# jalberse/RayTracingInOneWeekendInRust

Measured on AMD Instinct MI355X. Metric: Msamples/s (rays traced/s) + HBM GB/s vs roofline, showcase@1200x800x500spp, higher is better.
Workload: dtype f32; 1 GPU; C3 showcase 1200x800 500spp depth 50; scene=showcase, width=1200, height=800, spp=500, max_depth=50, parallelism=one GPU: the whole frame, exact_bvh=False

## Files before the change

### raytracinginoneweekendinrust_amd/__init__.py

```python
from __future__ import annotations

import ctypes as C
from dataclasses import dataclass, field
from typing import List, Optional, Sequence, Tuple

import numpy as np

from . import _capi
from ._capi import ASSET_DIR, RTError, check, lib
from .configs import CONFIGS, RenderConfig

__all__ = ["Camera", "CameraBasis", "BvhNode", "Renderer", "Scene", "SceneBuilder", "HittableList", "DeviceScene", "RenderConfig", "CONFIGS",
           "RTError", "tile", "device_count", "numeric_eval", "scene_background", "render_params", "ASSET_DIR",
           "set_option", "get_option", "options"]

Vec3 = Tuple[float, float, float]


class Scene:

    def __init__(self, desc_ptr, owner=None, name: str = ""):
        self._ptr = desc_ptr
        self._owner = owner
        self._lib_owned = owner is None
# ... 336 lines not shown
        yield done, (acc.copy() if last else acc / np.float32(done))


def render_multi(scenes: List[DeviceScene], camera: Camera, params,
                 out: Optional[np.ndarray] = None) -> Tuple[np.ndarray, dict]:
    if out is None:
        out = np.zeros((params.height, params.width, 3), dtype=np.float32)
    assert out.dtype == np.float32 and out.flags.c_contiguous and out.size == params.width * params.height * 3
    handles = (C.c_void_p * len(scenes))(*[s.handle for s in scenes])
    st = _capi.rt_stats()
    cam = camera.desc()
    check(lib.rt_render_multi(handles, len(scenes), C.byref(cam), C.byref(params),
                              out.ctypes.data_as(C.POINTER(C.c_float)), C.byref(st)), "rt_render_multi")
    return out, {"segments": st.segments, "samples": st.samples, "kernel_ms": st.kernel_ms}


def shard_floats(width: int, height: int, rank: int, n: int) -> int:
    return int(lib.rt_shard_floats(width, height, rank, n))


def shard_offset(width: int, height: int, rank: int, n: int) -> int:
    return int(lib.rt_shard_offset(width, height, rank, n))


def shard_mask(width: int, height: int, rank: int, n: int, device=None):
    import torch
    y = torch.arange(height, device=device).view(-1, 1) // 8
    x = torch.arange(width, device=device).view(1, -1) // 8
    return ((y * ((width + 7) // 8) + x) % n == rank).reshape(-1)


def shard_pack(d_image, width: int, height: int, rank: int, n: int, d_packed, stream: int = 0) -> None:
    check(lib.rt_shard_pack(C.c_void_p(d_image.data_ptr()), width, height, rank, n, C.c_void_p(d_packed.data_ptr()),
                            C.c_void_p(stream or None)), "rt_shard_pack")


IPC_HANDLE_BYTES = 72


def ipc_export(d_ptr: int, device: int) -> bytes:
    h = C.create_string_buffer(IPC_HANDLE_BYTES)
    check(lib.rt_ipc_export(C.c_void_p(d_ptr), device, h), "rt_ipc_export")
    return h.raw


def ipc_open(handle: bytes, device: int) -> int:
    p = C.c_void_p()
    check(lib.rt_ipc_open(C.create_string_buffer(handle, IPC_HANDLE_BYTES), device, C.byref(p)), "rt_ipc_open")
    return int(p.value)


def ipc_close(d_ptr: int, device: int) -> None:
    check(lib.rt_ipc_close(C.c_void_p(d_ptr), device), "rt_ipc_close")


def copy_async(d_dst: int, d_src: int, nbytes: int, stream: int = 0) -> None:
    check(lib.rt_copy_async(C.c_void_p(d_dst), C.c_void_p(d_src), nbytes, C.c_void_p(stream or None)),
          "rt_copy_async")


def shard_pull_unpack(peer_ptrs, width: int, height: int, d_image, stream: int = 0) -> None:
    n = len(peer_ptrs)
    arr = (C.c_void_p * n)(*[p or None for p in peer_ptrs])
    check(lib.rt_shard_pull_unpack(arr, width, height, n, C.c_void_p(d_image.data_ptr()), C.c_void_p(stream or None)),
          "rt_shard_pull_unpack")


def shard_unpack(d_packed_all, width: int, height: int, n: int, d_image, stream: int = 0) -> None:
    check(lib.rt_shard_unpack(C.c_void_p(d_packed_all.data_ptr()), width, height, n, C.c_void_p(d_image.data_ptr()),
                              C.c_void_p(stream or None)), "rt_shard_unpack")


def format_ppm(img: np.ndarray, device: int = 0) -> bytes:
    import torch
    h, w, _ = img.shape
    d_img = torch.from_numpy(np.ascontiguousarray(img, dtype=np.float32)).to(f"cuda:{device}")
    d_txt = torch.empty(12 * w * h, dtype=torch.uint8, device=f"cuda:{device}")
    n = C.c_uint64()
    stream = torch.cuda.current_stream(device).cuda_stream
    check(lib.rt_format_ppm(C.c_void_p(d_img.data_ptr()), w, h, C.c_void_p(d_txt.data_ptr()), d_txt.numel(),
                            C.byref(n), C.c_void_p(stream or None)), "rt_format_ppm")
    return f"P3\n{w} {h}\n255\n".encode() + bytes(d_txt[: n.value].cpu().numpy())


def quantize_srgb8(img: np.ndarray, device: int = 0) -> np.ndarray:
    import torch
    h, w, _ = img.shape
    d_img = torch.from_numpy(np.ascontiguousarray(img, dtype=np.float32)).to(f"cuda:{device}")
    d_u8 = torch.empty(3 * w * h, dtype=torch.uint8, device=f"cuda:{device}")
    stream = torch.cuda.current_stream(device).cuda_stream
    check(lib.rt_quantize_srgb8(C.c_void_p(d_img.data_ptr()), C.c_void_p(d_u8.data_ptr()), w, h,
                                C.c_void_p(stream or None)), "rt_quantize_srgb8")
    return d_u8.cpu().numpy().reshape(h, w, 3)


def tile(image_width: int, image_height: int, tile_width: int, tile_height: int) -> List[Tuple[int, int, int, int]]:
    n = C.c_uint32()
    check(lib.rt_tile_image(image_width, image_height, tile_width, tile_height, None, 0, C.byref(n)), "rt_tile_image")
    arr = (_capi.rt_tile * max(n.value, 1))()
    check(lib.rt_tile_image(image_width, image_height, tile_width, tile_height, arr, n.value, C.byref(n)),
          "rt_tile_image")
    return [(t.width, t.height, t.x_start, t.y_start) for t in arr[: n.value]]


def set_option(name: str, value: int) -> None:
    check(lib.rt_set_option(_capi.OPTIONS[name], int(value)), f"rt_set_option({name})")


def get_option(name: str) -> int:
    v = C.c_int64()
    check(lib.rt_get_option(_capi.OPTIONS[name], C.byref(v)), f"rt_get_option({name})")
    return v.value


class options:

    def __init__(self, **kw):
        self.kw = kw
        self.saved = {}

    def __enter__(self):
        for k, v in self.kw.items():
            self.saved[k] = get_option(k)
            set_option(k, v)
        return self

    def __exit__(self, *exc):
        for k, v in self.saved.items():
            set_option(k, v)
        return False


def device_count() -> int:
    n = C.c_int()
    check(lib.rt_device_count(C.byref(n)), "rt_device_count")
    return n.value


def scene_background(name: str) -> Vec3:
    rgb = (C.c_float * 3)()
    check(lib.rt_scene_background(name.encode(), rgb), "rt_scene_background")
    return (rgb[0], rgb[1], rgb[2])


def device_kat(op: int, cases) -> np.ndarray:
    a = np.ascontiguousarray(cases, dtype=np.float32)
    n = a.shape[0]
    out = np.zeros((n, 2), dtype=np.float32)
    check(lib.rt_device_kat(op, a.ctypes.data_as(C.POINTER(C.c_float)), out.ctypes.data_as(C.POINTER(C.c_float)), n),
          "rt_device_kat")
    return out


def numeric_eval(op: int, a: np.ndarray, b: Optional[np.ndarray] = None) -> np.ndarray:
    a = np.ascontiguousarray(a, dtype=np.float64)
    out = np.empty_like(a)
    bp = None
    if b is not None:
        b = np.ascontiguousarray(b, dtype=np.float64)
        bp = b.ctypes.data_as(C.POINTER(C.c_double))
    check(lib.rt_device_numeric_eval(op, a.ctypes.data_as(C.POINTER(C.c_double)), bp,
                                      out.ctypes.data_as(C.POINTER(C.c_double)), a.size), "rt_device_numeric_eval")
    return out
```

### raytracinginoneweekendinrust_amd/csrc/kernel.hip

```cpp
#include <hip/hip_runtime.h>
#include <stdint.h>
#include <stdio.h>
#include <math.h>
#include <stdlib.h>
#include <string.h>

#include <algorithm>
#include <atomic>
#include <mutex>
#include <string>
#include <vector>

#include "../../include/rt.h"
#include "../../include/rt_numeric_spec.h"
#include "common.hpp"
#include "device_scene.hpp"
#include "lower.hpp"

using rtdev::DevCamera;
using rtdev::DevEntry;
using rtdev::DevMaterial;
using rtdev::DevParams;
using rtdev::DevScene;
using rtdev::DevTexture;
using rtdev::f4;

#define RT_DEV __device__ __forceinline__

namespace {

constexpr float kInf = __builtin_inff();

enum ProfRegion : uint32_t {
    kPrRefill = 0, kPrSegment, kPrWorld, kPrRecord, kPrEmit, kPrScatter, kPrMarble, kPrStore,
    kPrChecker, kPrImage, kPrUnitSphere, kPrDielectric, kPrLambert, kPrMetal, kPrIso, kPrLog,
    kPrEntry0 = 16, kPrEntryLast = 43, kPrBvhTrip = 44, kPrLeafTest = 45, kPrBvhSetup = 46, kPrBvhPush = 47,
    kPrBvhPop = 48, kPrBvhCall = 49, kPrCount = 52
};
constexpr uint32_t kModeExact = 1u, kModeNoLeafBoxes = 2u, kModeNoPermLds = 32u, kModeW3 = 64u,
                   kModeNoPretest = 128u, kModeReplayRef = 1u << 16;
constexpr uint32_t kModeNoStream = 1u << 17;
constexpr uint32_t kModePruneAllExp = 1u << 20;
#if defined(RT_LEAF_AUDIT) || defined(RT_ABLATE)
constexpr bool kPruneAllExpBuild = true;
#else
constexpr bool kPruneAllExpBuild = false;
#endif
constexpr uint32_t kModeBlocksForward = 1u << 21;
constexpr uint32_t kModeW4 = 1u << 22;
[[maybe_unused]] constexpr uint32_t kModeMbShrink = 1u << 29;
constexpr uint32_t kTuneExact = kModeNoLeafBoxes | kModeNoPermLds | kModeW3 | kModeNoPretest | kModeReplayRef |
                                kModeNoStream | kModeBlocksForward | kModeW4 | (15u << 24);
constexpr uint32_t kTuneAccepted = kTuneExact
#if defined(RT_LEAF_AUDIT) || defined(RT_ABLATE)
                                   | kModePruneAllExp
#endif
#ifdef RT_LEAF_AUDIT
                                   | kModeMbShrink
#endif
#ifdef RT_ABLATE
                                   | (31u << 8)
#endif
#ifdef RT_EXP_STRIDE
                                   | (1u << 23)
#endif
    ;
#ifdef RT_ABLATE
constexpr uint32_t kAbLeaf2 = 1u << 8, kAbKeys2 = 1u << 9, kAbBvh2 = 1u << 10, kAbMedium2 = 1u << 11,
                   kAbGeom2 = 1u << 12;
#define ABLATE(bit, ...) do { if (mode & (bit)) { __VA_ARGS__ } } while (0)
#else
#define ABLATE(bit, ...) do { } while (0)
#endif
#ifdef RT_PROFILE_REGIONS
constexpr uint32_t kProfCopies = 64;
constexpr uint32_t kProfWords = 3 * kPrCount + 16;
__device__ unsigned long long g_prof[kProfCopies * kProfWords];
constexpr uint32_t kProfWaves = 8192;
__device__ unsigned long long g_wave_t[2 * kProfWaves];
constexpr uint32_t kTpBuckets = 4096, kTpTicks = 20000u;
__device__ unsigned long long g_tp_hist[kTpBuckets];
constexpr uint32_t kRoleEvents = 4096;
__device__ unsigned long long g_role_ev[2 * kRoleEvents];
__device__ unsigned g_role_n;
uint32_t g_prof_rows[2] = {0u, 0xffffffffu};
__device__ __forceinline__ void role_event(uint32_t what) {
    const unsigned i = atomicAdd(&g_role_n, 1u);
    if (i < kRoleEvents) {
        g_role_ev[2u * i] = __builtin_amdgcn_s_memrealtime();
        g_role_ev[2u * i + 1u] = what;
    }
}
__shared__ unsigned long long prof_lds[kProfWords];
__device__ __forceinline__ uint32_t trips_bin(uint32_t n) {
    return n == 0u ? 0u : n == 1u ? 1u : n == 2u ? 2u : n <= 4u ? 3u : n <= 8u ? 4u : n <= 16u ? 5u : n <= 32u ? 6u : 7u;
}
__device__ __forceinline__ void prof_init() {
    for (uint32_t i = threadIdx.x; i < kProfWords; i += blockDim.x) prof_lds[i] = 0u;
}
__device__ __forceinline__ void prof_flush() {
    unsigned long long* dst = g_prof + (blockIdx.x % kProfCopies) * kProfWords;
    for (uint32_t i = threadIdx.x; i < kProfWords; i += blockDim.x)
        if (prof_lds[i]) atomicAdd(&dst[i], prof_lds[i]);
}
#define PROF_T0(name) const uint64_t name = __builtin_amdgcn_s_memtime()
#define PROF_ADD(region, t0) prof_add((region), (t0))
__device__ __forceinline__ void prof_add(uint32_t region, uint64_t t0) {
    uint64_t dt = __builtin_amdgcn_s_memtime() - t0;
    uint64_t m = __ballot(1);
    if (__lane_id() == (uint32_t)__builtin_ctzll(m)) {
        prof_lds[region] += dt;
        prof_lds[kPrCount + region] += 1u;
        prof_lds[2 * kPrCount + region] += (uint64_t)__popcll(m);
    }
}
#define PROF_INIT() prof_init()
#define PROF_FLUSH() prof_flush()
#else
#define PROF_T0(name) do { } while (0)
#define PROF_ADD(region, t0) do { } while (0)
#define PROF_INIT() do { } while (0)
#define PROF_FLUSH() do { } while (0)
#endif
#ifdef RT_LEAF_AUDIT
struct LeafAudit {
    float o[3], d[3], tmin, closest, t, box[6], delta;
    uint32_t code, rank, best_rank;
};
constexpr uint32_t kAuditMax = 64;
__device__ unsigned g_audit_count;
__device__ LeafAudit g_audit[kAuditMax];
struct TravAudit {
    float o[3], d[3], tmin, tmax, fast_t, ref_t;
    uint32_t fast_code, ref_code, root;
};
__device__ unsigned g_trav_audit_count;
__device__ unsigned g_bounds_audit_count;
__device__ TravAudit g_trav_audit[kAuditMax];
#endif

struct V {
    float x, y, z;
};
#ifdef RT_DEBUG_PIXEL
constexpr uint32_t kDbgMax = 256;
__device__ uint32_t g_dbg[8 * kDbgMax];
__device__ unsigned g_dbg_n;
#ifndef RT_DEBUG_TRACE
#define RT_DEBUG_TRACE 1
#endif
#ifdef RT_DEBUG_INLINE
__device__ __forceinline__
#else
__device__ __noinline__
#endif
void dbg_put(uint32_t tag, uint32_t a, uint32_t b, uint32_t c, uint32_t d, uint32_t e,
                                     uint32_t f, uint32_t h) {
    const unsigned i = atomicAdd(&g_dbg_n, 1u);
    if (i < kDbgMax) {
        uint32_t* o = g_dbg + 8u * i;
        o[0] = tag; o[1] = a; o[2] = b; o[3] = c; o[4] = d; o[5] = e; o[6] = f; o[7] = h;
    }
}
#endif
RT_DEV V mk(float x, float y, float z) { return V{x, y, z}; }
RT_DEV V operator+(V a, V b) { return V{a.x + b.x, a.y + b.y, a.z + b.z}; }
RT_DEV V operator-(V a, V b) { return V{a.x - b.x, a.y - b.y, a.z - b.z}; }
RT_DEV V operator*(V a, V b) { return V{a.x * b.x, a.y * b.y, a.z * b.z}; }
RT_DEV V operator*(float s, V a) { return V{s * a.x, s * a.y, s * a.z}; }
RT_DEV V operator-(V a) { return V{-a.x, -a.y, -a.z}; }
RT_DEV V divs(V a, float s) { return V{a.x / s, a.y / s, a.z / s}; }
RT_DEV float dot(V a, V b) { return (a.x * b.x + a.y * b.y) + a.z * b.z; }
RT_DEV V cross(V a, V b) { return V{a.y * b.z - b.y * a.z, a.z * b.x - b.z * a.x, a.x * b.y - b.x * a.y}; }
RT_DEV float length(V a) { return __builtin_sqrtf(dot(a, a)); }
RT_DEV V normalize(V a) {
    float r = 1.0f / length(a);
    return V{a.x * r, a.y * r, a.z * r};
}
RT_DEV float rs_min(float a, float b) {
    if (a != a) return b;
    if (b != b) return a;
    return a < b ? a : b;
}
RT_DEV float rs_clamp(float x, float lo, float hi) {
    if (x < lo) x = lo;
    if (x > hi) x = hi;
    return x;
}
RT_DEV bool sign_negative(float x) { return (__float_as_uint(x) >> 31) != 0u; }
RT_DEV bool sign_negative_d(double x) { return (__double_as_longlong(x) >> 63) != 0; }
RT_DEV V xyz(f4 a) { return V{a.x, a.y, a.z}; }
[[maybe_unused]] RT_DEV float2 ld2(const f4* p, uint32_t row) {
    float2 v;
    __builtin_memcpy(&v, __builtin_assume_aligned(p + row, 16), sizeof(v));
    return v;
}
RT_DEV f4 ld4(const f4* p) {
    f4 v;
    __builtin_memcpy(&v, __builtin_assume_aligned(p, 16), sizeof(v));
    return v;
}
RT_DEV f4 ld4_at(const f4* base, uint32_t byte_off) {
    f4 v;
    __builtin_memcpy(&v, __builtin_assume_aligned(reinterpret_cast<const char*>(base) + byte_off, 16), sizeof(v));
    return v;
}
RT_DEV float ld1_at(const f4* base, uint32_t byte_off) {
    float v;
    __builtin_memcpy(&v, __builtin_assume_aligned(reinterpret_cast<const char*>(base) + byte_off, 4), sizeof(v));
    return v;
}
RT_DEV float2 ld2_at(const f4* base, uint32_t byte_off) {
    float2 v;
    __builtin_memcpy(&v, __builtin_assume_aligned(reinterpret_cast<const char*>(base) + byte_off, 8), sizeof(v));
    return v;
}
#ifndef RT_SCALAR_ENTRIES
#define RT_SCALAR_ENTRIES 1
#endif
#if RT_SCALAR_ENTRIES
#define RT_AS4 __attribute__((address_space(4)))
#else
#define RT_AS4
#endif
template <class T>
RT_DEV const RT_AS4 T* cst(const T* p) {
    return (const RT_AS4 T*)p;
}
RT_DEV f4 ld4c(const f4* p) {
    const RT_AS4 f4* q = cst(p);
    return f4{q->x, q->y, q->z, q->w};
}

struct Ray {
    V o, d;
    float time;
};
RT_DEV V at(const Ray& r, float t) { return r.o + t * r.d; }

struct Rng {
    uint32_t sample, pixel, d;
    uint32_t r0, r1, r2;
};
RT_DEV void philox(uint32_t& c0, uint32_t& c1, uint32_t& c2, uint32_t& c3, uint32_t k0, uint32_t k1) {
#pragma unroll
    for (int r = 0; r < 10; ++r) {
        const uint64_t p0 = (uint64_t)0xD2511F53u * c0, p1 = (uint64_t)0xCD9E8D57u * c2;
        const uint32_t lo0 = (uint32_t)p0, hi0 = (uint32_t)(p0 >> 32), lo1 = (uint32_t)p1, hi1 = (uint32_t)(p1 >> 32);
        uint32_t n0 = hi1 ^ c1 ^ k0, n2 = hi0 ^ c3 ^ k1;
        c0 = n0; c1 = lo1; c2 = n2; c3 = lo0;
        k0 += 0x9E3779B9u;
        k1 += 0xBB67AE85u;
    }
}
struct Key {
    uint32_t k0, k1;
};

#ifdef RT_PHILOX_CALL
__device__ __noinline__
#else
__device__ __forceinline__
#endif
uint4 philox_block(uint32_t c0, uint32_t c1, uint32_t c2, uint32_t k0, uint32_t k1) {
    uint32_t c3 = 0u;
    philox(c0, c1, c2, c3, k0, k1);
    return make_uint4(c0, c1, c2, c3);
}
#ifndef RT_RNG_UNIFORM
#ifdef RT_PHILOX_CALL
#define RT_RNG_UNIFORM 1
#else
#define RT_RNG_UNIFORM 0
#endif
#endif
// ... 546 lines not shown
            k = atomicCAS(&sl->key, ~0ull, key);
            if (k == ~0ull || k == key) return sl;
        }
    }
    return nullptr;
}
RT_DEV uint32_t hrpp_leaf_node(const DevScene& S, unsigned long long k) {
    uint32_t lo = 0, hi = S.hrpp_nkeys;
    while (lo < hi) {
        const uint32_t m = (lo + hi) >> 1;
        if (S.hrpp_keys[m] < k) lo = m + 1;
        else hi = m;
    }
    return lo < S.hrpp_nkeys && S.hrpp_keys[lo] == k ? S.hrpp_vals[lo] : 0xffffffffu;
}
RT_DEV bool bvh_hit_hrpp(const DevScene& S, uint32_t wrapper2, uint32_t pid, const Ray& r,
                                          const RayD& q, V inv, float tmin, float& closest, uint32_t& hit_code,
                                          uint32_t* stk) {
    rtdev::HrppSlot* tab = S.hrpp_tab + ((size_t)(pid - 1u) << S.hrpp_bits);
    uint32_t* cnt = S.hrpp_cnt + 4u * (pid - 1u);
    const unsigned long long key = hrpp_hash(r);
    const rtdev::HrppSlot* sl = S.hrpp_bits ? hrpp_find(tab, S.hrpp_bits, key, false) : nullptr;
    bool predicted = false;
    if (sl) {
        float c = closest;
        uint32_t code = 0u;
        bool any = false;
        for (uint32_t j = 0; j < rtdev::kHrppIds; ++j) {
            const uint32_t w = __hip_atomic_load(&sl->ids[j], __ATOMIC_RELAXED, __HIP_MEMORY_SCOPE_AGENT);
            if (w == 0xffffffffu) break;
            predicted = true;
            if (bvh_hit_reference(S, w, r, q, inv, tmin, c, code, stk)) any = true;
        }
        if (any) {
            atomicAdd(&cnt[0], 1u);
            closest = c;
            hit_code = code;
            return true;
        }
    }
    atomicAdd(&cnt[predicted ? 1u : 2u], 1u);
    const bool h = bvh_hit_reference(S, wrapper2, r, q, inv, tmin, closest, hit_code, stk);
    if (h && S.hrpp_bits) {
        const uint32_t leaf = hrpp_leaf_node(S, (unsigned long long)wrapper2 << 32 | hit_code);
        rtdev::HrppSlot* ins = leaf != 0xffffffffu ? hrpp_find(tab, S.hrpp_bits, key, true) : nullptr;
        bool ok = false;
        if (ins)
            for (uint32_t j = 0; j < rtdev::kHrppIds && !ok; ++j) {
                const uint32_t old = atomicCAS(&ins->ids[j], 0xffffffffu, leaf);
                ok = old == 0xffffffffu || old == leaf;
            }
        if (!ok) atomicAdd(&cnt[3], 1u);
    }
    return h;
}

[[maybe_unused]] RT_DEV float child_key(float x0, float y0, float z0, float x1, float y1, float z1, const Ray& r, V inv, float tmin,
                       float tmax_entry, float closest, bool prune, float dmi) {
    float te;
    bool go = slab(x0, y0, z0, x1, y1, z1, r, inv, tmin, tmax_entry, te);
    if (prune) te = te - dmi;
    if (go && prune) go = !(te > prune_bound(closest));
    return go ? (te < 3.4028235e38f ? te : 3.4028235e38f) : kInf;
}
typedef float pk2 __attribute__((ext_vector_type(2)));
RT_DEV pk2 pk(float a, float b) { return pk2{a, b}; }
RT_DEV void child_keys4_nf(f4 nx, f4 ny, f4 nz, f4 fx, f4 fy, f4 fz, const Ray& r, V inv, float tmin,
                           float tmax_entry, float pb, float dmi, float key[4]) {
    const pk2 ox = pk(r.o.x, r.o.x), oy = pk(r.o.y, r.o.y), oz = pk(r.o.z, r.o.z);
    const pk2 ix = pk(inv.x, inv.x), iy = pk(inv.y, inv.y), iz = pk(inv.z, inv.z);
#pragma unroll
    for (int h = 0; h < 2; ++h) {
        const pk2 tnx = ((h ? pk(nx.z, nx.w) : pk(nx.x, nx.y)) - ox) * ix, tfx = ((h ? pk(fx.z, fx.w) : pk(fx.x, fx.y)) - ox) * ix;
        const pk2 tny = ((h ? pk(ny.z, ny.w) : pk(ny.x, ny.y)) - oy) * iy, tfy = ((h ? pk(fy.z, fy.w) : pk(fy.x, fy.y)) - oy) * iy;
        const pk2 tnz = ((h ? pk(nz.z, nz.w) : pk(nz.x, nz.y)) - oz) * iz, tfz = ((h ? pk(fz.z, fz.w) : pk(fz.x, fz.y)) - oz) * iz;
#pragma unroll
        for (int e = 0; e < 2; ++e) {
            const float lo = __builtin_fmaxf(__builtin_fmaxf(tnx[e], tny[e]), __builtin_fmaxf(tnz[e], tmin));
            const float hi = __builtin_fminf(__builtin_fminf(tfx[e], tfy[e]), __builtin_fminf(tfz[e], tmax_entry));
            const float te = lo - dmi;
            const bool go = lo <= hi && te <= pb;
            key[2 * h + e] = go ? __builtin_fminf(te, 3.4028235e38f) : kInf;
        }
    }
}
RT_DEV void leaf_intervals2_nf(float2 nx, float2 ny, float2 nz, float2 fx, float2 fy, float2 fz, const Ray& r,
                               V inv, float delta, float lo[2], float hi[2]) {
    const bool sx = inv.x < 0.0f, sy = inv.y < 0.0f, sz = inv.z < 0.0f;
    const float pxs = r.o.x + delta, pys = r.o.y + delta, pzs = r.o.z + delta;
    const float mxs = r.o.x - delta, mys = r.o.y - delta, mzs = r.o.z - delta;
    const float anx = sx ? mxs : pxs, afx = sx ? pxs : mxs, sny = sy ? mys : pys, afy = sy ? pys : mys;
    const float anz = sz ? mzs : pzs, afz = sz ? pzs : mzs;
    const pk2 ix = pk(inv.x, inv.x), iy = pk(inv.y, inv.y), iz = pk(inv.z, inv.z);
    const pk2 tnx = (pk(nx.x, nx.y) - pk(anx, anx)) * ix, tfx = (pk(fx.x, fx.y) - pk(afx, afx)) * ix;
    const pk2 tny = (pk(ny.x, ny.y) - pk(sny, sny)) * iy, tfy = (pk(fy.x, fy.y) - pk(afy, afy)) * iy;
    const pk2 tnz = (pk(nz.x, nz.y) - pk(anz, anz)) * iz, tfz = (pk(fz.x, fz.y) - pk(afz, afz)) * iz;
#pragma unroll
    for (int e = 0; e < 2; ++e) {
        lo[e] = __builtin_fmaxf(__builtin_fmaxf(tnx[e], tny[e]), tnz[e]);
        hi[e] = __builtin_fminf(__builtin_fminf(tfx[e], tfy[e]), tfz[e]);
    }
}
RT_DEV bool leaf_interval_may_hit(float lo, float hi, float tmin, float closest) {
    if (lo > prune_bound(closest)) return false;
    if (tmin > 0.0f && hi < tmin * (1.0f - 0x1p-19f)) return false;
    return !(lo - hi > (__builtin_fabsf(lo) + __builtin_fabsf(hi)) * 0x1p-19f);
}
RT_DEV void sort2(float& ta, uint32_t& ca, float& tb, uint32_t& cb) {
    const bool sw = tb < ta;
    const float a = ta, b = tb;
    const uint32_t x = ca, y = cb;
    ta = sw ? b : a;
    tb = sw ? a : b;
    ca = sw ? y : x;
    cb = sw ? x : y;
}
struct Trav {
    uint32_t cur, sp, best_rank;
    float tmax_entry;
    bool any;
    uint32_t pend;
};
constexpr uint32_t kNoNode = 0xffffffffu;
RT_DEV void trav_audit(const DevScene& S, const f4* wrapper, uint32_t root, const Ray& r, V inv, float tmin,
                       const Trav& tv, float closest, uint32_t hit_code, uint32_t* stk) {
#ifdef RT_LEAF_AUDIT
    const bool any = tv.any;
    float c2 = tv.tmax_entry;
    uint32_t h2 = 0u;
    bool a2 = bvh_hit_reference(S, __float_as_uint(ld4c(wrapper + 7).z), r, to_d(r), inv, tmin, c2, h2, stk);
    bool same = a2 == any && (!any || (__float_as_uint(c2) == __float_as_uint(closest) && h2 == hit_code));
    if (!same) {
        unsigned i_ = atomicAdd(&g_trav_audit_count, 1u);
        if (i_ < kAuditMax) {
            TravAudit& A = g_trav_audit[i_];
            A.o[0] = r.o.x; A.o[1] = r.o.y; A.o[2] = r.o.z;
            A.d[0] = r.d.x; A.d[1] = r.d.y; A.d[2] = r.d.z;
            A.tmin = tmin; A.tmax = tv.tmax_entry;
            A.fast_t = any ? closest : kInf; A.ref_t = a2 ? c2 : kInf;
            A.fast_code = any ? hit_code : 0xffffffffu; A.ref_code = a2 ? h2 : 0xffffffffu;
            A.root = root;
        }
    }
#endif
}
#ifndef RT_SUSP_MIN_TRIPS
#define RT_SUSP_MIN_TRIPS 2
#endif
constexpr uint32_t kSuspMinTrips = RT_SUSP_MIN_TRIPS;
#ifndef RT_LEAF_Q
#define RT_LEAF_Q 8
#endif

template <int kKind, uint32_t kF, bool kSusp>
RT_DEV bool bvh_run(const DevScene& S, float delta, const f4* wrapper, const Ray& r, V inv, float tmin, float& closest,
                    uint32_t& hit_code, uint32_t* stk, uint32_t mode, Trav& tv, uint32_t susp);
constexpr uint32_t kRayFast = 0u, kRayHandOver = 1u, kRayNoHit = 2u;
#ifndef RT_TRI_ZERO_DIR_FAST
#define RT_TRI_ZERO_DIR_FAST 1
#endif
template <int kKind, uint32_t kF>
RT_DEV uint32_t ray_route(const Ray& r, V inv, float tmax_entry, const f4* wrapper, uint32_t mode) {
    const float ax = __builtin_fabsf(inv.x), ay = __builtin_fabsf(inv.y), az = __builtin_fabsf(inv.z);
    const bool ofin = __builtin_fabsf(r.o.x) < kInf && __builtin_fabsf(r.o.y) < kInf && __builtin_fabsf(r.o.z) < kInf;
    const bool tnum = tmax_entry == tmax_entry;
    if (ax > 0.0f && ax < kInf && ay > 0.0f && ay < kInf && az > 0.0f && az < kInf && ofin && tnum) return kRayFast;
    if constexpr ((kF & kFTri) != 0u && (kKind == 3 || (kKind == 0 && RT_TRI_ZERO_DIR_FAST))) {
        if ((__float_as_uint(ld4c(wrapper + 7).w) & rtdev::kBvhTriOnly) != 0u &&
            !(kPruneAllExpBuild && (mode & kModePruneAllExp))) {
            if (r.o.x != r.o.x || r.o.y != r.o.y || r.o.z != r.o.z || r.d.x != r.d.x || r.d.y != r.d.y ||
                r.d.z != r.d.z)
                return kRayNoHit;
            const bool dfin =
                __builtin_fabsf(r.d.x) < kInf && __builtin_fabsf(r.d.y) < kInf && __builtin_fabsf(r.d.z) < kInf;
            if (dfin && ofin && tnum) return kRayFast;
        }
    }
    return kRayHandOver;
}

template <uint32_t kF>
RT_DEV bool bvh_hit_nan_tmax(const DevScene& S, const f4* wrapper, const Ray& r, float tmin, float& closest,
                             uint32_t& hit_code) {
    const f4* T = S.nodes + (size_t)__float_as_uint(ld4c(wrapper + 7).y) * rtdev::kBvhNodeF4;
    const uint32_t n = __float_as_uint(ld1_at(T, 0u));
    const float nan = __uint_as_float(0x7fc00000u);
    bool any = false;
    float best = 0.0f;
    uint32_t best_code = 0u;
    auto test = [&](uint32_t i, float tmax, float& t) {
        const uint32_t idx = rtdev::leaf_index(__float_as_uint(ld1_at(T, 16u + 4u * i)));
        return tri_t(ld4(S.tri + 3 * (size_t)idx), ld4(S.tri + 3 * (size_t)idx + 1), ld4(S.tri + 3 * (size_t)idx + 2), r,
                     tmin, tmax, t);
    };
    for (uint32_t i = 0; i < n;) {
        const uint32_t e = __float_as_uint(ld1_at(T, 16u + 4u * i));
        const bool pair = (e & rtdev::kDfsPairLeft) != 0u && i + 1u < n;
        float tl = 0.0f, tr = 0.0f;
        const bool hl = test(i, nan, tl);
        const bool hr = pair && test(i + 1u, hl ? tl : nan, tr);
        if (hl || hr) {
            const float t = hr ? tr : tl;
            if (!any || !(best < t)) {
                any = true;
                best = t;
                best_code = __float_as_uint(ld1_at(T, 16u + 4u * (hr ? i + 1u : i))) & ~rtdev::kDfsPairLeft;
            }
        }
        i += pair ? 2u : 1u;
    }
    if (!any) return false;
    closest = best;
    hit_code = best_code;
    return true;
}

#ifndef RT_PEEL_WRAPPER
#define RT_PEEL_WRAPPER 1
#endif
constexpr bool kPeelWrapper = RT_PEEL_WRAPPER;
template <int kKind, uint32_t kF = kFAll>
RT_DEV bool bvh_hit(const DevScene& S, float delta, uint32_t root, const Ray& r, float tmin, float& closest,
                    uint32_t& hit_code, uint32_t* stk, uint32_t mode, bool& replay) {
    PROF_T0(pcall);
    PROF_T0(psetup);
    const f4* wrapper = S.nodes + (size_t)root * rtdev::kBvhNodeF4;
    const V inv = mk(1.0f / r.d.x, 1.0f / r.d.y, 1.0f / r.d.z);
    if constexpr (kKind == 1 || kKind == 2) {
        const RayD q = to_d(r);
        const uint32_t w2 = __float_as_uint(ld4c(wrapper + 7).z);
        if constexpr (kKind == 2) {
            const uint32_t pid = __float_as_uint(S.nodes2[4 * (size_t)w2 + 3].z);
            if (pid) return bvh_hit_hrpp(S, w2, pid, r, q, inv, tmin, closest, hit_code, stk);
        }
        return bvh_hit_reference(S, w2, r, q, inv, tmin, closest, hit_code, stk);
    }
    {
        const uint32_t route = ray_route<kKind, kF>(r, inv, closest, wrapper, mode);
        if (route == kRayNoHit) return false;
        if constexpr (kKind == 3) {
            if (route == kRayHandOver) {
                if constexpr ((kF & kFTri) != 0u) {
                    const bool fin = __builtin_fabsf(r.o.x) < kInf && __builtin_fabsf(r.o.y) < kInf &&
                                     __builtin_fabsf(r.o.z) < kInf && __builtin_fabsf(r.d.x) < kInf &&
                                     __builtin_fabsf(r.d.y) < kInf && __builtin_fabsf(r.d.z) < kInf;
                    if (closest != closest && fin &&
                        (__float_as_uint(ld4c(wrapper + 7).w) & rtdev::kBvhTriOnly) != 0u &&
                        !(kPruneAllExpBuild && (mode & kModePruneAllExp)))
                        return bvh_hit_nan_tmax<kF>(S, wrapper, r, tmin, closest, hit_code);
                }
                return bvh_hit_reference(S, __float_as_uint(ld4c(wrapper + 7).z), r, to_d(r), inv, tmin, closest, hit_code,
                                         stk);
            }
        }
        if (route == kRayHandOver) {
            replay = true;
            return false;
        }
    }
    PROF_ADD(kPrBvhSetup, psetup);
    Trav tv{root, 0u, 0u, closest, false, kNoNode};
    if constexpr (kPeelWrapper) {
        const f4 w0 = ld4c(wrapper), w1 = ld4c(wrapper + 1), w2 = ld4c(wrapper + 2), w3 = ld4c(wrapper + 3),
                 w4 = ld4c(wrapper + 4), w5 = ld4c(wrapper + 5), w6 = ld4c(wrapper + 6), w7 = ld4c(wrapper + 7);
        const bool prune = (__float_as_uint(w7.w) & rtdev::kBvhPrunable) != 0u ||
                           (kPruneAllExpBuild && (mode & kModePruneAllExp));
        const float dmi = delta * fmaxf(fmaxf(__builtin_fabsf(inv.x), __builtin_fabsf(inv.y)), __builtin_fabsf(inv.z));
        const bool sx = inv.x < 0.0f, sy = inv.y < 0.0f, sz = inv.z < 0.0f;
        const float tnx = ((sx ? w3.x : w0.x) - r.o.x) * inv.x, tfx = ((sx ? w0.x : w3.x) - r.o.x) * inv.x;
        const float tny = ((sy ? w4.x : w1.x) - r.o.y) * inv.y, tfy = ((sy ? w1.x : w4.x) - r.o.y) * inv.y;
        const float tnz = ((sz ? w5.x : w2.x) - r.o.z) * inv.z, tfz = ((sz ? w2.x : w5.x) - r.o.z) * inv.z;
        const float lo = __builtin_fmaxf(__builtin_fmaxf(tnx, tny), __builtin_fmaxf(tnz, tmin));
        const float hi = __builtin_fminf(__builtin_fminf(tfx, tfy), __builtin_fminf(tfz, closest));
        const float te = lo - (prune ? dmi : 0.0f);
        if (lo <= hi && te <= (prune ? prune_bound(closest) : kInf)) {
            tv.cur = __float_as_uint(w6.x);
            bvh_run<kKind, kF, false>(S, delta, wrapper, r, inv, tmin, closest, hit_code, stk, mode, tv, 0u);
        }
    } else {
        bvh_run<kKind, kF, false>(S, delta, wrapper, r, inv, tmin, closest, hit_code, stk, mode, tv, 0u);
    }
    const bool any = tv.any;
    PROF_ADD(kPrBvhCall, pcall);
    trav_audit(S, wrapper, root, r, inv, tmin, tv, closest, hit_code, stk);
    return any;
}

#ifndef RT_POP_PREFETCH
#define RT_POP_PREFETCH 0
#endif
template <uint32_t kF>
constexpr bool kPopPrefetch = RT_POP_PREFETCH && (kF & (kFTri | kFDeep)) == 0u;
template <int kKind, uint32_t kF, bool kSusp>
RT_DEV bool bvh_run(const DevScene& S, float delta, const f4* wrapper, const Ray& r, V inv, float tmin, float& closest,
                    uint32_t& hit_code, uint32_t* stk, uint32_t mode, Trav& tv, uint32_t susp) {
    const float tmax_entry = tv.tmax_entry;
    const bool prune = (__float_as_uint(ld4c(wrapper + 7).w) & rtdev::kBvhPrunable) != 0u ||
                       (kPruneAllExpBuild && (mode & kModePruneAllExp));
    const float dmi = delta * fmaxf(fmaxf(__builtin_fabsf(inv.x), __builtin_fabsf(inv.y)), __builtin_fabsf(inv.z));
    const bool leaf_boxes = prune && !(mode & kModeNoLeafBoxes);
    [[maybe_unused]] const uint32_t hnx = inv.x < 0.0f ? 48u : 0u, hny = inv.y < 0.0f ? 64u : 16u,
                                    hnz = inv.z < 0.0f ? 80u : 32u;
    bool any = tv.any;
    uint32_t best_rank = tv.best_rank, sp = tv.sp, cur = tv.cur, pend = tv.pend;
    constexpr bool kPostpone = (kF & kFTri) != 0u && kKind == 0;
    const uint32_t tq = (mode >> 24) & 15u;
    const uint32_t lq = !kPostpone ? 0u : (tq == 15u ? 0u : (tq ? tq : (uint32_t)RT_LEAF_Q));
    bool finished = true;
    [[maybe_unused]] uint32_t trips = 0;
#ifdef RT_PROFILE_REGIONS
    uint32_t visits = 0;
#endif
    for (;;) {
        if constexpr (kSusp) {
            if (trips >= kSuspMinTrips && (uint32_t)__popcll(__ballot(1)) <= susp) {
                finished = false;
                break;
            }
            ++trips;
        }
        uint32_t lnode = kNoNode;
        bool popnext = false, do_int;
        if constexpr (kPostpone) {
            const bool cur_leaf = cur != kNoNode && (cur & rtdev::kLeafNodeFlag) != 0u;
            const bool has_pend = pend != kNoNode;
            bool leafphase = true;
            if (lq) {
                const bool can_adv = cur != kNoNode && (!cur_leaf || !has_pend);
                const uint32_t n_act = (uint32_t)__popcll(__ballot(1)), n_pend = (uint32_t)__popcll(__ballot(has_pend));
                leafphase = __ballot(can_adv) == 0ull || n_pend * 16u >= lq * n_act;
            }
            if (leafphase) {
                if (has_pend) {
                    lnode = pend;
                    pend = kNoNode;
                } else if (cur_leaf) {
                    lnode = cur;
                    popnext = true;
                }
            } else if (cur_leaf && !has_pend) {
                pend = cur;
                popnext = true;
            }
            do_int = lnode == kNoNode && !popnext && cur != kNoNode && !cur_leaf;
        } else {
            const bool cur_leaf = (cur & rtdev::kLeafNodeFlag) != 0u;
            lnode = cur_leaf ? cur : kNoNode;
            do_int = !cur_leaf;
        }
        uint32_t onx, ony, onz;
        if constexpr ((kF & kFTri) != 0u) {
            onx = hnx;
            ony = hny;
            onz = hnz;
        } else {
            uint32_t msx, msy, msz;
            asm volatile("v_ashrrev_i32 %0, 31, %1" : "=v"(msx) : "v"(inv.x));
            asm volatile("v_ashrrev_i32 %0, 31, %1" : "=v"(msy) : "v"(inv.y));
            asm volatile("v_ashrrev_i32 %0, 31, %1" : "=v"(msz) : "v"(inv.z));
            onx = msx & 48u;
            ony = (msy & 48u) + 16u;
            onz = (msz & 48u) + 32u;
        }
#ifdef RT_LEAF_AUDIT
        {
            const uint32_t vis = lnode != kNoNode ? lnode : cur;
            if ((vis != kNoNode && (vis & ~rtdev::kLeafNodeFlag) >= S.num_nodes) || sp > S.stack_depth + S.spill_depth) {
                atomicAdd(&g_bounds_audit_count, 1u);
                break;
            }
        }
#endif
#ifdef RT_PROFILE_REGIONS
        ++visits;
#endif
        [[maybe_unused]] uint32_t pf_node = 0u;
        [[maybe_unused]] float pf_t = 0.0f;
        if constexpr (kPopPrefetch<kF>) {
            const uint32_t top = (sp > 0u ? sp - 1u : 0u) * 128u;
            pf_node = stk[top];
            pf_t = __uint_as_float(stk[top + 64u]);
        }
        PROF_T0(pt);
        if (lnode != kNoNode) {
            const uint32_t nbo = (lnode & ~rtdev::kLeafNodeFlag) * (rtdev::kBvhNodeF4 * 16u);
            const f4* nd = S.nodes;
            const float2 nx2 = ld2_at(nd, nbo + onx), ny2 = ld2_at(nd, nbo + ony), nz2 = ld2_at(nd, nbo + onz),
                         fx2 = ld2_at(nd, nbo + (onx ^ 48u)), fy2 = ld2_at(nd, nbo + (ony ^ 80u)),
                         fz2 = ld2_at(nd, nbo + (onz ^ 112u)), chs = ld2_at(nd, nbo + 96u), rks = ld2_at(nd, nbo + 112u);
            float tmr = tmax_entry, nt = 0.0f;
            bool nh = false;
            uint32_t ncode = 0u, nrank = 0u;
            const uint32_t nleaf = __float_as_uint(chs.y) == rtdev::kChildEmpty ? 1u : 2u;
            float llo[2] = {-kInf, -kInf}, lhi[2] = {kInf, kInf};
            if (leaf_boxes) leaf_intervals2_nf(nx2, ny2, nz2, fx2, fy2, fz2, r, inv, delta, llo, lhi);
            for (uint32_t k = 0; k < nleaf; ++k) {
                const uint32_t lcode = __float_as_uint(k ? chs.y : chs.x), rank = __float_as_uint(k ? rks.y : rks.x);
#ifdef RT_LEAF_AUDIT
                const float2 bx0 = ld2(S.nodes + nbo / 16u, 0), by0 = ld2(S.nodes + nbo / 16u, 1),
                             bz0 = ld2(S.nodes + nbo / 16u, 2), bx1 = ld2(S.nodes + nbo / 16u, 3),
                             by1 = ld2(S.nodes + nbo / 16u, 4), bz1 = ld2(S.nodes + nbo / 16u, 5);
                const float x0 = k ? bx0.y : bx0.x, y0 = k ? by0.y : by0.x, z0 = k ? bz0.y : bz0.x;
                const float x1 = k ? bx1.y : bx1.x, y1 = k ? by1.y : by1.x, z1 = k ? bz1.y : bz1.x;
#endif
                const float bound = tmr < closest ? tmr : closest;
                if (!leaf_boxes || leaf_interval_may_hit(k ? llo[1] : llo[0], k ? lhi[1] : lhi[0], tmin, bound)) {
                    PROF_T0(pl);
                    const float cap = closest < kInf ? __uint_as_float(__float_as_uint(closest) + 1u) : kInf;
                    float c = tmr < cap ? tmr : cap;
                    uint32_t code = 0u;
                    const RayD q = to_d(r);
                    ABLATE(kAbLeaf2, float c2 = c; uint32_t h2 = 0u;
                           if (leaf_hit<kF>(S, lcode, r, q, tmin, c2, h2) && h2 == 0x7fffffffu) c = -1.0f;);
                    bool hit;
                    if constexpr (kLeafEmbed<kF>) {
                        const uint32_t ltype = rtdev::leaf_type(lcode);
                        const uint32_t lo = nbo + 4u * k;
                        if (ltype == rtdev::kLeafSphere) {
                            const f4 sp{ld1_at(nd, lo + 8u), ld1_at(nd, lo + 24u), ld1_at(nd, lo + 40u), ld1_at(nd, lo + 104u)};
                            float ts;
                            hit = sphere_t(sp, q, tmin, c, ts);
                            if (hit) {
                                c = ts;
                                code = lcode;
                            }
                        } else if (ltype == rtdev::kLeafCube) {
                            hit = cube_hit<(kF & kFTri) == 0u>(S, rtdev::leaf_index(lcode), ld1_at(nd, lo), ld1_at(nd, lo + 16u),
                                                               ld1_at(nd, lo + 32u), ld1_at(nd, lo + 48u), ld1_at(nd, lo + 64u),
                                                               ld1_at(nd, lo + 80u), r, inv, tmin, c, code);
                        } else {
                            hit = leaf_hit<kF, (kF & kFTri) == 0u, false, true>(S, lcode, r, q, tmin, c, code, inv);
                        }
                    } else {
                        hit = leaf_hit<kF, (kF & kFTri) == 0u>(S, lcode, r, q, tmin, c, code, inv);
                    }
                    if (hit) {
                        const uint32_t rk = rank + (rtdev::leaf_type(lcode) == rtdev::kLeafCube
                                                        ? rtdev::leaf_index(code) - rtdev::leaf_index(lcode)
                                                        : 0u);
                        if (!nh || !(nt < c)) {
                            nh = true;
                            nt = c;
                            ncode = code;
                            nrank = rk;
                        }
                        tmr = c;
                    }
                    PROF_ADD(kPrLeafTest, pl);
                } else {
                    LEAF_AUDIT(lcode, rank, x0, y0, z0, x1, y1, z1);
                }
            }
            if (nh && (nt < closest || (nt == closest && nrank > best_rank))) {
                closest = nt;
                best_rank = nrank;
                hit_code = ncode;
                any = true;
            }
        }
        float t0 = kInf, t1 = kInf, t2 = kInf, t3 = kInf;
        uint32_t c0 = rtdev::kChildEmpty, c1 = rtdev::kChildEmpty, c2 = rtdev::kChildEmpty, c3 = rtdev::kChildEmpty;
        if (do_int) {
            const uint32_t nbo = cur * (rtdev::kBvhNodeF4 * 16u);
            const f4* nd = S.nodes;
            const f4 nx = ld4_at(nd, nbo + onx), ny = ld4_at(nd, nbo + ony), nz = ld4_at(nd, nbo + onz),
                     fx = ld4_at(nd, nbo + (onx ^ 48u)), fy = ld4_at(nd, nbo + (ony ^ 80u)),
                     fz = ld4_at(nd, nbo + (onz ^ 112u)), chf = ld4_at(nd, nbo + 96u);
            c0 = __float_as_uint(chf.x);
            c1 = __float_as_uint(chf.y);
            c2 = __float_as_uint(chf.z);
            c3 = __float_as_uint(chf.w);
            ABLATE(kAbKeys2, const f4 mnx = inv.x < 0.0f ? fx : nx; const f4 mxx = inv.x < 0.0f ? nx : fx;
                   const f4 mny = inv.y < 0.0f ? fy : ny; const f4 mxy = inv.y < 0.0f ? ny : fy;
                   const f4 mnz = inv.z < 0.0f ? fz : nz; const f4 mxz = inv.z < 0.0f ? nz : fz;
                   float k2 = child_key(mnx.x, mny.x, mnz.x, mxx.x, mxy.x, mxz.x, r, inv, tmin, tmax_entry,
                                                  closest, prune, dmi) +
                                        child_key(mnx.y, mny.y, mnz.y, mxx.y, mxy.y, mxz.y, r, inv, tmin, tmax_entry,
                                                  closest, prune, dmi) +
                                        child_key(mnx.z, mny.z, mnz.z, mxx.z, mxy.z, mxz.z, r, inv, tmin, tmax_entry,
                                                  closest, prune, dmi) +
                                        child_key(mnx.w, mny.w, mnz.w, mxx.w, mxy.w, mxz.w, r, inv, tmin, tmax_entry,
                                                  closest, prune, dmi);
                   if (k2 == -1.0f) c0 = 0u;);
            float key[4];
            child_keys4_nf(nx, ny, nz, fx, fy, fz, r, inv, tmin, tmax_entry, prune ? prune_bound(closest) : kInf,
                           prune ? dmi : 0.0f, key);
            t0 = key[0];
            t1 = key[1];
            t2 = key[2];
            t3 = key[3];
        }
        PROF_ADD(kPrBvhTrip, pt);
        PROF_T0(pp);
        auto push = [&](uint32_t node, float t) {
            if (!(kF & kFDeep) || sp < S.stack_depth) {
                stk[sp * 128u] = node;
                stk[sp * 128u + 64u] = __float_as_uint(t);
            } else {
                uint32_t* g = S.stack_spill +
                              (((size_t)blockIdx.x * S.spill_depth + (sp - S.stack_depth)) * 64u + threadIdx.x) * 2u;
                g[0] = node;
                g[1] = __float_as_uint(t);
            }
            sp += 1u;
        };
        sort2(t0, c0, t1, c1);
        sort2(t2, c2, t3, c3);
        sort2(t0, c0, t2, c2);
        sort2(t1, c1, t3, c3);
        sort2(t1, c1, t2, c2);
        if (t0 != kInf) {
            if (t3 != kInf) push(c3, t3);
            if (t2 != kInf) push(c2, t2);
            if (t1 != kInf) push(c1, t1);
            cur = c0;
            if constexpr (!kPostpone) {
                PROF_ADD(kPrBvhPush, pp);
                continue;
            }
        } else if (!kPostpone || do_int) {
            popnext = true;
        }
        PROF_ADD(kPrBvhPush, pp);
        PROF_T0(ppop);
        if (popnext) {
            bool found = false;
            [[maybe_unused]] bool first = true;
            while (sp > 0u) {
                sp -= 1u;
                uint32_t cand;
                float tenter;
                if (kPopPrefetch<kF> && first) {
                    cand = pf_node;
                    tenter = pf_t;
                    first = false;
                } else if (!(kF & kFDeep) || sp < S.stack_depth) {
                    cand = stk[sp * 128u];
                    tenter = __uint_as_float(stk[sp * 128u + 64u]);
                } else {
                    const uint32_t* g = S.stack_spill +
                                        (((size_t)blockIdx.x * S.spill_depth + (sp - S.stack_depth)) * 64u + threadIdx.x) * 2u;
                    cand = g[0];
                    tenter = __uint_as_float(g[1]);
                }
                if (!prune || !(tenter > prune_bound(closest))) {
                    cur = cand;
                    found = true;
                    break;
                }
            }
            if (!found) {
                if constexpr (!kPostpone) {
                    PROF_ADD(kPrBvhPop, ppop);
                    break;
                } else {
                    cur = kNoNode;
                }
            }
        }
        PROF_ADD(kPrBvhPop, ppop);
        if constexpr (kPostpone) {
            if (cur == kNoNode && pend == kNoNode) break;
        }
    }
    tv = Trav{cur, sp, best_rank, tmax_entry, any, pend};
#ifdef RT_PROFILE_REGIONS
    {
        const uint32_t b = trips_bin(visits);
        uint32_t m = visits;
        for (int off = 32; off > 0; off >>= 1) {
            uint32_t o = __shfl_xor(m, off);
            m = o > m ? o : m;
        }
        const uint32_t first = (uint32_t)__builtin_ctzll(__ballot(1));
        for (uint32_t bin = 0; bin < 8u; ++bin) {
            const uint32_t n = (uint32_t)__popcll(__ballot(b == bin));
            if (__lane_id() == first && n) prof_lds[3u * kPrCount + bin] += n;
        }
        if (__lane_id() == first) prof_lds[3u * kPrCount + 8u + trips_bin(m)] += 1u;
    }
#endif
    return finished;
}

RT_DEV Ray apply_op(f4 op, Ray r) {
    if (op.w == 0.0f) {
        r.o = r.o - xyz(op);
    } else {
        float s = op.x, c = op.y;
        r.o = mk(c * r.o.x - s * r.o.z, r.o.y, s * r.o.x + c * r.o.z);
        r.d = mk(c * r.d.x - s * r.d.z, r.d.y, s * r.d.x + c * r.d.z);
    }
    return r;
}

RT_DEV void spheres_surely_missed2(f4 s0, f4 s1, const Ray& r, float a, bool& m0, bool& m1) {
    const pk2 ocx = pk(r.o.x, r.o.x) - pk(s0.x, s1.x), ocy = pk(r.o.y, r.o.y) - pk(s0.y, s1.y),
              ocz = pk(r.o.z, r.o.z) - pk(s0.z, s1.z);
    const pk2 dx = pk(r.d.x, r.d.x), dy = pk(r.d.y, r.d.y), dz = pk(r.d.z, r.d.z), a2 = pk(a, a);
    const pk2 hb = (ocx * dx + ocy * dy) + ocz * dz;
    const pk2 oc2 = (ocx * ocx + ocy * ocy) + ocz * ocz;
    const pk2 rad = pk(s0.w, s1.w);
    const pk2 r2 = rad * rad;
    const pk2 hb2 = hb * hb;
    const pk2 disc = hb2 - a2 * (oc2 - r2);
    const pk2 m = hb2 + a2 * (oc2 + r2);
    const pk2 lim = pk(-0x1p-16f, -0x1p-16f) * m;
    m0 = m[0] > 0x1p-100f && disc[0] < lim[0];
    m1 = m[1] > 0x1p-100f && disc[1] < lim[1];
}

template <uint32_t kF>
constexpr bool kUniformEntries = (kF & kFTri) != 0u || (kF & (kFBvh | kFRuns)) == 0u;
template <uint32_t kF>
RT_DEV uint32_t uni(uint32_t v) {
    if constexpr (kUniformEntries<kF>) return __builtin_amdgcn_readfirstlane(v);
    return v;
}
template <uint32_t kF>
RT_DEV Ray apply_op_u(f4 op, Ray r) {
    if (__uint_as_float(uni<kF>(__float_as_uint(op.w))) == 0.0f) {
        r.o = r.o - xyz(op);
    } else {
        float s = op.x, c = op.y;
        r.o = mk(c * r.o.x - s * r.o.z, r.o.y, s * r.o.x + c * r.o.z);
        r.d = mk(c * r.d.x - s * r.d.z, r.d.y, s * r.d.x + c * r.d.z);
    }
    return r;
}
constexpr uint32_t kRunPretestMin = 8u;
template <int kKind, uint32_t kF>
RT_DEV bool entry_geom_hit(const DevScene& S, float delta, const DevEntry* E, Ray r, float tmin, float& closest,
                           uint32_t& hit_code, uint32_t* stk, uint32_t mode, bool& replay) {
    uint32_t ntf = uni<kF>(cst(E)->ntf);
    for (uint32_t i = 0; i < ntf; ++i) r = apply_op_u<kF>(ld4c(&E->tf[i]), r);
    const uint32_t kind = uni<kF>(cst(E)->kind);
    if (kind == rtdev::kEntSphereRun) {
        const uint32_t first = uni<kF>(cst(E)->payload), n = uni<kF>(cst(E)->pad[0]);
        const RayD q = to_d(r);
        const bool pretest = (kF & kFRuns) && n >= kRunPretestMin && !(mode & kModeNoPretest);
        bool any = false;
        auto test = [&](uint32_t i, f4 sp, bool missed) {
            float t;
            if (missed) {
#ifdef RT_LEAF_AUDIT
                if (sphere_roots(sp, q).ok) atomicAdd(&g_audit_count, 1u);
#endif
                return;
            }
            if (sphere_t(sp, q, tmin, closest, t)) {
                closest = t;
                hit_code = rtdev::leaf_code(rtdev::kLeafSphere, first + i);
                any = true;
            }
        };
        uint32_t i = 0;
        if (pretest) {
            const float a = (r.d.x * r.d.x + r.d.y * r.d.y) + r.d.z * r.d.z;
            for (; i + 1u < n; i += 2u) {
                const f4 s0 = ld4c(S.sph + first + i), s1 = ld4c(S.sph + first + i + 1u);
                bool m0, m1;
                spheres_surely_missed2(s0, s1, r, a, m0, m1);
                test(i, s0, m0);
                test(i + 1u, s1, m1);
            }
        }
        for (; i < n; ++i) {
            const f4 sp = ld4c(S.sph + first + i);
            test(i, sp, pretest && sphere_surely_missed(sp, r));
        }
        return any;
    }
    if (kind == rtdev::kEntRectRun) {
        const uint32_t first = uni<kF>(cst(E)->payload), n = uni<kF>(cst(E)->pad[0]);
        bool any = false;
        for (uint32_t i = 0; i < n; ++i) {
            const uint32_t idx = first + i;
            const f4 r0 = ld4c(S.rect + 2 * idx), r1 = ld4c(S.rect + 2 * idx + 1);
            float t;
            bool h;
            if constexpr (kUniformEntries<kF>) {
                const uint32_t axis = __builtin_amdgcn_readfirstlane(__float_as_uint(r1.y));
                if (axis == 0u)
                    h = side_t(r0.x, r.o.z, r.d.z, r.o.x, r.d.x, r.o.y, r.d.y, r0.y, r0.z, r0.w, r1.x, tmin, closest, t);
                else if (axis == 1u)
                    h = side_t(r0.x, r.o.y, r.d.y, r.o.x, r.d.x, r.o.z, r.d.z, r0.y, r0.z, r0.w, r1.x, tmin, closest, t);
                else
                    h = side_t(r0.x, r.o.x, r.d.x, r.o.y, r.d.y, r.o.z, r.d.z, r0.y, r0.z, r0.w, r1.x, tmin, closest, t);
            } else {
                h = rect_t(r0, r1, r, tmin, closest, t);
            }
            if (h) {
                closest = t;
                hit_code = rtdev::leaf_code(rtdev::kLeafRect, idx);
                any = true;
            }
        }
        return any;
    }
    if (kind == rtdev::kEntBvh) {
        if constexpr ((kF & kFBvh) == 0u) {
            return false;
        } else {
            ABLATE(kAbBvh2, float c2 = closest; uint32_t h2 = 0u; bool rp = false;
                   if (bvh_hit<kKind, kF>(S, delta, cst(E)->payload, r, tmin, c2, h2, stk, mode, rp) && h2 == 0x7fffffffu)
                       closest = -1.0f;);
            return bvh_hit<kKind, kF>(S, delta, uni<kF>(cst(E)->payload), r, tmin, closest, hit_code, stk, mode,
                                            replay);
        }
    }
    if constexpr (kUniformEntries<kF>) {
        const uint32_t code = __builtin_amdgcn_readfirstlane(cst(E)->payload);
        if (rtdev::leaf_type(code) == rtdev::kLeafRect) {
            const uint32_t idx = rtdev::leaf_index(code);
            const f4 r0 = ld4c(S.rect + 2 * idx), r1 = ld4c(S.rect + 2 * idx + 1);
            const uint32_t axis = __builtin_amdgcn_readfirstlane(__float_as_uint(r1.y));
            float t;
            bool h;
            if (axis == 0u)
                h = side_t(r0.x, r.o.z, r.d.z, r.o.x, r.d.x, r.o.y, r.d.y, r0.y, r0.z, r0.w, r1.x, tmin, closest, t);
            else if (axis == 1u)
                h = side_t(r0.x, r.o.y, r.d.y, r.o.x, r.d.x, r.o.z, r.d.z, r0.y, r0.z, r0.w, r1.x, tmin, closest, t);
            else
                h = side_t(r0.x, r.o.x, r.d.x, r.o.y, r.d.y, r.o.z, r.d.z, r0.y, r0.z, r0.w, r1.x, tmin, closest, t);
            if (h) {
                closest = t;
                hit_code = code;
            }
            return h;
        }
    }
    RayD q = to_d(r);
    ABLATE(kAbGeom2, float c2 = closest; uint32_t h2 = 0u;
           if (leaf_hit<kF | kFLeafRM>(S, cst(E)->payload, r, q, tmin, c2, h2) && h2 == 0x7fffffffu) closest = -1.0f;);
    return leaf_hit<kF | kFLeafRM, false, true>(S, uni<kF>(cst(E)->payload), r, q, tmin, closest, hit_code);
}

#ifndef RT_MEDIUM_FIRST
#define RT_MEDIUM_FIRST 1
#endif
template <uint32_t kF>
constexpr bool kMediumFirst = RT_MEDIUM_FIRST && (kF & kFBvh) != 0u && (kF & kFMarble) != 0u && (kF & kFTri) == 0u;
template <uint32_t kF>
RT_DEV float medium_first_estimate(const DevScene& S, const DevEntry* E, Ray r, const Rng& g, const Key& k) {
    const uint32_t ntf = cst(E)->ntf;
    for (uint32_t i = 0; i < ntf; ++i) r = apply_op_u<kF>(ld4c(&E->tf[i]), r);
    const DevEntry* B = S.entries + cst(E)->payload;
    Ray rb = r;
    const uint32_t bn = cst(B)->ntf;
    for (uint32_t i = 0; i < bn; ++i) rb = apply_op_u<kF>(ld4c(&B->tf[i]), rb);
    const f4 s = ld4c(S.sph + rtdev::leaf_index(cst(B)->payload));
    const V oc = rb.o - xyz(s);
    const float a = dot(rb.d, rb.d), hb = dot(oc, rb.d), cq = dot(oc, oc) - s.w * s.w;
    const float disc = hb * hb - a * cq;
    if (!(disc >= 0.0f)) return kInf;
    const float sq = __builtin_sqrtf(disc);
    const float r2 = (sq - hb) / a;
    float t1 = (-hb - sq) / a;
    if (t1 < 0.001f) t1 = 0.001f;
    if (!(t1 < r2)) return kInf;
    const float len = length(r.d);
    Rng p = g;
    const float hd = cst(E)->neg_inv_density * __logf(std01(p, k));
    if (!(hd < (r2 - t1) * len * (1.0f - 0x1p-10f))) return kInf;
    return (t1 + hd / len) * (1.0f + 0x1p-8f) + 0x1p-16f;
}

template <int kKind, uint32_t kF>
RT_DEV bool medium_hit(const DevScene& S, float delta, const DevEntry* E, Ray r, float tmin, float tmax, Rng& g,
                       const Key& k, float& t_out, uint32_t* stk, uint32_t mode, bool& replay,
                       float vbound = kInf) {
    uint32_t ntf = uni<kF>(cst(E)->ntf);
    for (uint32_t i = 0; i < ntf; ++i) r = apply_op_u<kF>(ld4c(&E->tf[i]), r);
    const DevEntry* B = S.entries + uni<kF>(cst(E)->payload);
    float t1 = kInf, t2 = kInf;
    const uint32_t bkind = uni<kF>(cst(B)->kind), bcode = uni<kF>(cst(B)->payload);
    if (bkind == rtdev::kEntGeom && rtdev::leaf_type(bcode) == rtdev::kLeafSphere) {
        Ray rb = r;
        uint32_t bn = uni<kF>(cst(B)->ntf);
        for (uint32_t i = 0; i < bn; ++i) rb = apply_op_u<kF>(ld4c(&B->tf[i]), rb);
        Roots R = sphere_roots(ld4c(S.sph + rtdev::leaf_index(bcode)), to_d(rb));
        ABLATE(kAbMedium2, Roots R2 = sphere_roots(ld4(S.sph + rtdev::leaf_index(cst(B)->payload)), to_d(rb));
               if (R2.r1 == -1.0) t1 = -1.0f;);
        if (!sphere_select(R, -kInf, kInf, t1)) return false;
        if (!sphere_select(R, t1 + 0.0001f, kInf, t2)) return false;
    } else if ((kF & kFTri) == 0u && bkind == rtdev::kEntGeom && rtdev::leaf_type(bcode) == rtdev::kLeafCube) {
        Ray rb = r;
        uint32_t bn = uni<kF>(cst(B)->ntf);
        for (uint32_t i = 0; i < bn; ++i) rb = apply_op_u<kF>(ld4c(&B->tf[i]), rb);
        const uint32_t idx = rtdev::leaf_index(bcode);
        const f4 s0 = ld4c(S.rect + 2 * idx);
        const float y1 = ld4c(S.rect + 2 * idx + 1).x, z1 = ld4c(S.rect + 2 * idx + 5).x;
        const float x0 = s0.y, x1 = s0.z, y0 = s0.w, z0 = s0.x;
        const float ox = rb.o.x, oy = rb.o.y, oz = rb.o.z, dx = rb.d.x, dy = rb.d.y, dz = rb.d.z;
        float tt[6];
        uint32_t in = 0u;
        {
            const float num[6] = {z0 - oz, z1 - oz, y0 - oy, y1 - oy, x0 - ox, x1 - ox};
            const float den[6] = {dz, dz, dy, dy, dx, dx};
#pragma unroll
            for (int f = 0; f < 6; ++f) tt[f] = num[f] / den[f];
        }
        auto side = [&](int f, float oa, float da, float ob, float db, float a0, float a1, float b0, float b1) {
            const float x = oa + tt[f] * da, y = ob + tt[f] * db;
            if (!(x < a0 || x > a1 || y < b0 || y > b1)) in |= 1u << f;
        };
        side(0, ox, dx, oy, dy, x0, x1, y0, y1);
        side(1, ox, dx, oy, dy, x0, x1, y0, y1);
        side(2, ox, dx, oz, dz, x0, x1, z0, z1);
        side(3, ox, dx, oz, dz, x0, x1, z0, z1);
        side(4, oy, dy, oz, dz, y0, y1, z0, z1);
        side(5, oy, dy, oz, dz, y0, y1, z0, z1);
        auto pick = [&](float lo, float& closest) {
            bool any = false;
#pragma unroll
            for (int f = 0; f < 6; ++f)
                if (((in >> f) & 1u) && !(tt[f] < lo || tt[f] > closest)) {
                    closest = tt[f];
                    any = true;
                }
            return any;
        };
        if (!pick(-kInf, t1)) return false;
        if (!pick(t1 + 0.0001f, t2)) return false;
    } else {
        uint32_t dummy;
        if (!entry_geom_hit<kKind, kF>(S, delta, B, r, -kInf, t1, dummy, stk, mode, replay)) return false;
        if (!entry_geom_hit<kKind, kF>(S, delta, B, r, t1 + 0.0001f, t2, dummy, stk, mode, replay)) return false;
    }
    if (t1 < tmin) t1 = tmin;
    if (t2 > tmax) t2 = tmax;
    if (t1 >= t2) return false;
    if (t1 < 0.0f) t1 = 0.0f;
    float ray_length = length(r.d);
    float distance_inside = (t2 - t1) * ray_length;
    PROF_T0(pl);
    float hit_distance = cst(E)->neg_inv_density * rt_logf(std01(g, k));
    PROF_ADD(kPrLog, pl);
    if constexpr (kKind == 0 && kMediumFirst<kF>) {
        if (vbound < kInf) {
            const float t2v = t2 > vbound ? vbound : t2;
            if (!(t1 < t2v) || hit_distance > (t2v - t1) * ray_length) replay = true;
        }
    }
    if (hit_distance > distance_inside) return false;
    t_out = t1 + hit_distance / ray_length;
    return true;
}

struct Rec {
    V p, n;
    float t, u, v;
    bool front;
    uint32_t mat;
};
__device__ __noinline__ void sphere_uv(V p, float& u, float& v) {
    const float PI = 3.14159265358979323846f;
    const float TWO_PI = 2.0f * PI;
    float theta = rt_acosf(-p.y);
    float phi = rt_atan2f(-p.z, p.x) + PI;
    u = phi / TWO_PI;
// ... 236 lines not shown
            return mk(s, s, s);
        }
        PROF_T0(pi);
        uint32_t w = T->b, h = T->c;
        float uu = rs_clamp(u, 0.0f, 1.0f);
        float vv = 1.0f - rs_clamp(v, 0.0f, 1.0f);
        uint32_t i = rt_f32_to_u32_sat(uu * (float)w);
        uint32_t j = rt_f32_to_u32_sat(vv * (float)h);
        if (i >= w) i = w - 1u;
        if (j >= h) j = h - 1u;
        const uint8_t* px = S.texels + T->a + ((size_t)j * w + i) * 3u;
        const float cs = 1.0f / 255.0f;
        V texel = mk((float)px[0] * cs, (float)px[1] * cs, (float)px[2] * cs);
        PROF_ADD(kPrImage, pi);
        return texel;
    }
}

RT_DEV V reflect(V v, V n) { return v - (2.0f * dot(v, n)) * n; }
RT_DEV V refract(V uv, V n, float eta) {
    float cos_t = rs_min(dot(-uv, n), 1.0f);
    V r_perp = eta * (uv + cos_t * n);
    V r_par = (-__builtin_sqrtf(__builtin_fabsf(1.0f - dot(r_perp, r_perp)))) * n;
    return r_par + r_perp;
}
RT_DEV bool near_zero(V v) {
    const float eps = 1.1920929e-07f;
    return __builtin_fabsf(v.x) < eps && __builtin_fabsf(v.y) < eps && __builtin_fabsf(v.z) < eps;
}
template <bool kTurb = false>
RT_DEV bool scatter(const DevScene& S, const DevMaterial& m, const Ray& r, const Rec& rec, Rng& g, const Key& k,
                    V& att, Ray& sc, uint32_t tex = 0u, double turb = 0.0, bool att_later = false) {
    sc.o = rec.p;
    sc.time = r.time;
    V rs = mk(0.0f, 0.0f, 0.0f);
    if (m.kind == rtdev::kMatLambertian || m.kind == rtdev::kMatMetal || m.kind == rtdev::kMatIsotropic) {
        PROF_T0(pu);
        rs = in_unit_sphere(g, k);
        PROF_ADD(kPrUnitSphere, pu);
#ifdef RT_DEBUG_PIXEL
        if ((RT_DEBUG_TRACE & 2) && g.pixel == RT_DEBUG_PIXEL && g.sample == RT_DEBUG_SAMPLE)
            dbg_put(2u, __float_as_uint(rs.x), __float_as_uint(rs.y), __float_as_uint(rs.z), g.d, g.r0, g.r1, g.r2);
#endif
    }
    if (m.kind == rtdev::kMatLambertian) {
        PROF_T0(pb);
        V dir = rec.n + normalize(rs);
        if (near_zero(dir)) dir = rec.n;
        sc.d = dir;
        if (!att_later) att = tex_value<kTurb>(S, kTurb ? tex : m.tex, rec.u, rec.v, rec.p, turb);
        PROF_ADD(kPrLambert, pb);
        return true;
    }
    if (m.kind == rtdev::kMatMetal) {
        PROF_T0(pt);
        V reflected = reflect(normalize(r.d), rec.n);
        V dir = reflected + m.fuzz * rs;
        sc.d = dir;
        att = mk(m.albedo[0], m.albedo[1], m.albedo[2]);
        PROF_ADD(kPrMetal, pt);
        return dot(dir, rec.n) > 0.0f;
    }
    if (m.kind == rtdev::kMatDielectric) {
        PROF_T0(pd);
        att = mk(1.0f, 1.0f, 1.0f);
        float ratio = rec.front ? 1.0f / m.ior : m.ior;
        V ud = normalize(r.d);
        float cos_t = rs_min(dot(-ud, rec.n), 1.0f);
        float sin_t = __builtin_sqrtf(1.0f - cos_t * cos_t);
        bool cannot = ratio * sin_t > 1.0f;
        bool refl = cannot;
        if (!cannot) {
            float q = (1.0f - ratio) / (1.0f + ratio);
            float r0 = q * q;
            float x = 1.0f - cos_t;
            float x2 = x * x;
            float refl_p = r0 + (1.0f - r0) * (x * (x2 * x2));
            refl = refl_p > std01(g, k);
        }
        sc.d = refl ? reflect(ud, rec.n) : refract(ud, rec.n, ratio);
        PROF_ADD(kPrDielectric, pd);
        return true;
    }
    if (m.kind == rtdev::kMatIsotropic) {
        PROF_T0(ps);
        sc.d = rs;
        if (!att_later) att = tex_value<kTurb>(S, kTurb ? tex : m.tex, rec.u, rec.v, rec.p, turb);
        PROF_ADD(kPrIso, ps);
        return true;
    }
    return false;
}

RT_DEV void start_sample(const DevCamera& C, const DevParams& P, const Key& k, uint32_t x, uint32_t y,
                         uint32_t pixel, uint32_t sample, Rng& g, Ray& ray) {
    g.sample = sample;
    g.pixel = pixel;
    g.d = 0u;
    float u = ((float)x + std01(g, k)) / (float)(P.width - 1u);
    float v = ((float)y + std01(g, k)) / (float)(P.height - 1u);
    V rd = C.lens_radius * in_unit_disk(g, k);
    V cu = mk(C.u[0], C.u[1], C.u[2]), cv = mk(C.v[0], C.v[1], C.v[2]);
    V org = mk(C.origin[0], C.origin[1], C.origin[2]);
    V offset = rd.x * cu + rd.y * cv;
    ray.o = org + offset;
    V llc = mk(C.llc[0], C.llc[1], C.llc[2]);
    V hor = mk(C.horizontal[0], C.horizontal[1], C.horizontal[2]);
    V ver = mk(C.vertical[0], C.vertical[1], C.vertical[2]);
    ray.d = llc + u * hor + v * ver - org - offset;
    float v01 = from_1_2(next_u32(g, k)) - 1.0f;
    ray.time = v01 * C.time_scale + C.time_low;
}

static inline uint32_t batch_group(uint64_t units, uint32_t waves) {
    const uint64_t g = units / ((uint64_t)(waves ? waves : 1u) * 32u);
    return g < 4u ? 4u : g > 64u ? 64u : (uint32_t)g;
}
constexpr uint32_t kPermLdsMax = 4u * 9u * 256u;
#ifndef RT_MT_LDS
#define RT_MT_LDS 1
#endif
constexpr uint32_t kMtLdsMax = 2048u;
struct ChunkParams {
    uint32_t sample0;
    uint32_t samples;
    uint32_t units;
    uint32_t guide;
    uint32_t fast_grid;
    uint32_t nslots;
    uint32_t group;
    uint32_t blocks;
};

template <int kKind, uint32_t kF>
RT_DEV bool world_hit(const DevScene& S, float delta, const Ray& r, Rng& g, const Key& k, float& t_hit,
                      uint32_t& hit_entry, uint32_t& hit_code, uint32_t* stk, uint32_t mode, bool& replay) {
    float closest = kInf;
    float cb = kInf;
    if constexpr (kKind == 0 && kMediumFirst<kF>) {
        if (S.mb_entry < S.num_top) {
            cb = medium_first_estimate<kF>(S, S.entries + S.mb_entry, r, g, k);
#ifdef RT_LEAF_AUDIT
            if (mode & kModeMbShrink) cb *= 0.5f;
#endif
            const float md = fminf(fabsf(r.d.x), fminf(fabsf(r.d.y), fabsf(r.d.z)));
            const float b = cb * (1.0f + 0x1p-18f) + (delta + delta) / md;
            if (b < kInf) closest = b; else cb = kInf;
        }
    }
    bool any = false;
    for (uint32_t e = 0; e < S.num_top; ++e) {
        const DevEntry* E = S.entries + e;
        PROF_T0(pe);
        if (uni<kF>(cst(E)->kind) == rtdev::kEntMedium) {
            float t, vb = kInf;
            if constexpr (kKind == 0 && kMediumFirst<kF>) {
                if (e == S.mb_entry && closest > cb) {
                    closest = kInf;
                    any = false;
                    vb = cb;
                }
            }
            const bool mh = medium_hit<kKind, kF>(S, delta, E, r, 0.001f, closest, g, k, t, stk, mode, replay, vb);
            if (vb < kInf && !mh) replay = true;
            if (mh) {
                closest = t;
                hit_entry = e;
                hit_code = rtdev::leaf_code(rtdev::kLeafMedium, 0);
                any = true;
            }
        } else {
            uint32_t code;
            if (entry_geom_hit<kKind, kF>(S, delta, E, r, 0.001f, closest, code, stk, mode, replay)) {
                hit_entry = e;
                hit_code = code;
                any = true;
            }
        }
        PROF_ADD(e < kPrEntryLast - kPrEntry0 ? kPrEntry0 + e : kPrEntryLast, pe);
    }
    t_hit = closest;
    return any;
}

struct Walk {
    uint32_t pos;
    bool resume;
    bool any;
    float closest;
    uint32_t hit_entry, hit_code;
    Trav tv;
};
template <uint32_t kF>
RT_DEV void world_walk(const DevScene& S, float delta, const Ray& ray, Rng& g, const Key& k, Walk& w, bool active,
                       uint32_t* stk, uint32_t mode, bool& replay, uint32_t susp) {
    for (uint32_t e = 0; e < S.num_top; ++e) {
        if (!(active && w.pos == e)) continue;
        PROF_T0(pe);
        const DevEntry* E = S.entries + e;
        const uint32_t kind = uni<kF>(cst(E)->kind);
        if (kind == rtdev::kEntMedium) {
            float t;
            if (medium_hit<0, kF>(S, delta, E, ray, 0.001f, w.closest, g, k, t, stk, mode, replay)) {
                w.closest = t;
                w.hit_entry = e;
                w.hit_code = rtdev::leaf_code(rtdev::kLeafMedium, 0);
                w.any = true;
            }
            w.pos = e + 1u;
        } else if ((kF & kFBvh) && kind == rtdev::kEntBvh) {
            Ray r = ray;
            const uint32_t ntf = uni<kF>(cst(E)->ntf);
            for (uint32_t i = 0; i < ntf; ++i) r = apply_op_u<kF>(ld4c(&E->tf[i]), r);
            const uint32_t root = uni<kF>(cst(E)->payload);
            const f4* wrapper = S.nodes + (size_t)root * rtdev::kBvhNodeF4;
            const V inv = mk(1.0f / r.d.x, 1.0f / r.d.y, 1.0f / r.d.z);
            if (!w.resume) {
                const uint32_t route = ray_route<0, kF>(r, inv, w.closest, wrapper, mode);
                if constexpr (RT_TRI_ZERO_DIR_FAST && (kF & kFTri) != 0u) {
                    if (route == kRayNoHit) {
                        w.pos = e + 1u;
                        continue;
                    }
                }
                if (route != kRayFast) {
                    replay = true;
                    w.pos = S.num_top + 1u;
                    continue;
                }
                w.tv = Trav{root, 0u, 0u, w.closest, false, kNoNode};
            }
            if (bvh_run<0, kF, true>(S, delta, wrapper, r, inv, 0.001f, w.closest, w.hit_code, stk, mode, w.tv, susp)) {
                trav_audit(S, wrapper, root, r, inv, 0.001f, w.tv, w.closest, w.hit_code, stk);
                if (w.tv.any) {
                    w.hit_entry = e;
                    w.any = true;
                }
                w.pos = e + 1u;
                w.resume = false;
            } else {
                w.resume = true;
            }
        } else {
            uint32_t code;
            if (entry_geom_hit<0, kF>(S, delta, E, ray, 0.001f, w.closest, code, stk, mode, replay)) {
                w.hit_entry = e;
                w.hit_code = code;
                w.any = true;
            }
            w.pos = e + 1u;
        }
        PROF_ADD(e < kPrEntryLast - kPrEntry0 ? kPrEntry0 + e : kPrEntryLast, pe);
    }
}

struct ItemPool {
    uint32_t batch, next, end;
    bool exhausted;
};
struct TraceCounters {
    unsigned batch;
    unsigned replay_count;
    unsigned replay_pull;
    unsigned batch_full;
    unsigned fast_done;
    unsigned stream_abort;
    unsigned long long fast_segments;
};
struct ReplayItem {
    uint32_t pixel, sample;
};
constexpr unsigned long long kReplayFree = ~0ull;
constexpr size_t kCamOffset = 256;
RT_DEV void replay_publish(ReplayItem* list, uint32_t idx, uint32_t pixel, uint32_t sample) {
    __hip_atomic_store(reinterpret_cast<unsigned long long*>(list + idx),
                       (unsigned long long)pixel | ((unsigned long long)sample << 32), __ATOMIC_RELAXED,
                       __HIP_MEMORY_SCOPE_AGENT);
}
RT_DEV unsigned long long replay_peek(const ReplayItem* list, uint32_t idx) {
    return __hip_atomic_load(reinterpret_cast<const unsigned long long*>(list + idx), __ATOMIC_RELAXED,
                             __HIP_MEMORY_SCOPE_AGENT);
}
RT_DEV ReplayItem replay_take(const ReplayItem* list, uint32_t idx) {
    const unsigned long long v = replay_peek(list, idx);
    __hip_atomic_store(reinterpret_cast<unsigned long long*>(const_cast<ReplayItem*>(list) + idx), kReplayFree,
                       __ATOMIC_RELAXED, __HIP_MEMORY_SCOPE_AGENT);
    return ReplayItem{(uint32_t)v, (uint32_t)(v >> 32)};
}
constexpr uint32_t kReplayCap = 1u << 20;
#ifndef RT_SBUF_NT
#define RT_SBUF_NT 2
#endif
template <uint32_t kF = kFAll>
RT_DEV void sbuf_store(float* o, V L) {
    if constexpr (RT_SBUF_NT == 1 || (RT_SBUF_NT == 2 && (kF & kFBvh) != 0u)) {
        __builtin_nontemporal_store(L.x, o);
        __builtin_nontemporal_store(L.y, o + 1);
        __builtin_nontemporal_store(L.z, o + 2);
    } else {
        o[0] = L.x;
        o[1] = L.y;
        o[2] = L.z;
    }
}
constexpr uint32_t kReplayNone = 0xffffffffu;
constexpr uint32_t kStreamWaves = 512;
constexpr unsigned long long kStreamTimeoutTicks = 1000000000ull;
RT_DEV uint32_t replay_claim(TraceCounters* ctr, const ReplayItem* list, uint32_t fast_grid) {
    const uint32_t i = atomicAdd(&ctr->replay_pull, 1u);
    const unsigned long long t0 = __builtin_amdgcn_s_memrealtime();
    for (;;) {
        const bool done = __hip_atomic_load(&ctr->fast_done, __ATOMIC_ACQUIRE, __HIP_MEMORY_SCOPE_AGENT) >= fast_grid;
        const uint32_t n = __hip_atomic_load(&ctr->replay_count, __ATOMIC_RELAXED, __HIP_MEMORY_SCOPE_AGENT);
        if (i < n) {
            if (i >= kReplayCap) return kReplayNone;
            if (replay_peek(list, i) != kReplayFree) return i;
        } else if (done) {
            return kReplayNone;
        }
        if (__builtin_amdgcn_s_memrealtime() - t0 > kStreamTimeoutTicks) {
            atomicExch(&ctr->stream_abort, 1u);
            return kReplayNone;
        }
        for (int z = 0; z < 4; ++z)
            __builtin_amdgcn_s_sleep(127);
    }
}
RT_DEV bool take_sample(ItemPool& pool, bool want, const DevCamera& C, const DevParams& P, const ChunkParams& Q,
                        const Key& k, unsigned* counter, const ReplayItem* list, uint32_t list_n,
                        TraceCounters* ctr, uint32_t stream_grid, float* sbuf,
                        uint32_t lane, uint32_t& slot, uint32_t& s_local, V& L, V& T, uint32_t& depth, Rng& g,
                        Ray& ray) {
    bool got = false;
#ifdef RT_LEAF_AUDIT
    if (__ballot(1) != ~0ull) atomicAdd(&g_bounds_audit_count, 1u);
#endif
    for (;;) {
        unsigned long long need = __ballot(want && !got);
        if (need == 0ull || pool.exhausted) break;
        if (pool.next == pool.end) {
            const bool leader = lane == 0u;
            uint32_t bt = 0, cnt = 64u;
            if (list && stream_grid) {
                uint32_t lim = 1u;
                if (leader) {
                    const uint32_t n = __hip_atomic_load(&ctr->replay_count, __ATOMIC_RELAXED, __HIP_MEMORY_SCOPE_AGENT);
                    const uint32_t pl = __hip_atomic_load(&ctr->replay_pull, __ATOMIC_RELAXED, __HIP_MEMORY_SCOPE_AGENT);
                    lim += (n > pl ? n - pl : 0u) / gridDim.x;
                }
                lim = __builtin_amdgcn_readfirstlane(lim);
                if (64u - (uint32_t)__popcll(need) >= lim) break;
// ... 91 lines not shown
}

template <uint32_t kF = kFAll>
RT_DEV bool finish_segment(const DevScene& S, const DevParams& P, const ChunkParams& Q, const Key& k,
                           float* __restrict__ sbuf, bool any, uint32_t he, uint32_t hc, float t, Ray& ray, V& L, V& T,
                           uint32_t& depth, Rng& g, uint32_t slot, uint32_t s_local) {
    PROF_T0(pg);
#ifdef RT_DEBUG_PIXEL
    if ((RT_DEBUG_TRACE & 1) && g.pixel == RT_DEBUG_PIXEL && g.sample == RT_DEBUG_SAMPLE)
        dbg_put(1u, depth, g.d, g.r0, g.r1, g.r2, any ? hc : 0xffffffffu, __float_as_uint(t));
#endif
    bool done;
    if (!any) {
        L = L + T * mk(P.bg[0], P.bg[1], P.bg[2]);
        done = true;
    } else {
        Rec rec;
        PROF_T0(pc);
        make_record<kF>(S, he, hc, t, ray, rec);
        PROF_ADD(kPrRecord, pc);
        const DevMaterial m = S.mats[rec.mat];
        PROF_T0(pm);
        V em = m.kind == rtdev::kMatLight ? tex_value(S, m.tex, rec.u, rec.v, rec.p) : mk(0.0f, 0.0f, 0.0f);
        L = L + T * em;
        PROF_ADD(kPrEmit, pm);
        V att;
        Ray sc;
        PROF_T0(ps);
        bool scattered = scatter(S, m, ray, rec, g, k, att, sc);
        PROF_ADD(kPrScatter, ps);
#ifdef RT_DEBUG_PIXEL
        if ((RT_DEBUG_TRACE & 4) && g.pixel == RT_DEBUG_PIXEL && g.sample == RT_DEBUG_SAMPLE)
            dbg_put(3u, rec.mat, m.kind, __float_as_uint(sc.d.x), __float_as_uint(sc.d.y), __float_as_uint(sc.d.z), g.d,
                    __float_as_uint(rec.n.y));
#endif
        if (scattered) {
            T = T * att;
            ray = sc;
            depth -= 1u;
            done = depth == 0u;
        } else {
            done = true;
        }
    }
    if (done) {
        sbuf_store<kF>(sbuf + ((size_t)s_local * Q.nslots + slot) * 3u, L);
    }
    PROF_ADD(kPrSegment, pg);
    return done;
}

template <uint32_t kF>
RT_DEV bool shade_marble(const DevScene& S, const DevParams& P, const ChunkParams& Q, const Key& k,
                         float* __restrict__ sbuf, bool shade, bool any, uint32_t he, uint32_t hc, float t, Ray& ray,
                         V& L, V& T, uint32_t& depth, Rng& g, uint32_t slot, uint32_t s_local) {
    bool marble = false, mlight = false, scattered = false, done = false;
    V mp = mk(0.0f, 0.0f, 0.0f);
    uint32_t tab = 0u;
    float mscale = 0.0f;
    if (shade && !any) {
        L = L + T * mk(P.bg[0], P.bg[1], P.bg[2]);
        done = true;
    } else if (shade) {
        Rec rec;
        PROF_T0(pc);
        make_record<kF>(S, he, hc, t, ray, rec);
        PROF_ADD(kPrRecord, pc);
        const DevMaterial m = S.mats[rec.mat];
        uint32_t tex = m.tex;
        if (m.kind == rtdev::kMatLight || m.kind == rtdev::kMatLambertian || m.kind == rtdev::kMatIsotropic) {
            tex = tex_resolve(S, m.tex, rec.p);
            const DevTexture& tx = S.texs[tex];
            marble = tx.kind == rtdev::kTexMarble;
            tab = tx.a;
            mscale = tx.scale;
        }
        mp = rec.p;
        mlight = m.kind == rtdev::kMatLight;
        if (!(marble && mlight)) {
            const V em = mlight ? tex_value<true>(S, tex, rec.u, rec.v, rec.p, 0.0) : mk(0.0f, 0.0f, 0.0f);
            L = L + T * em;
        }
        V att;
        Ray sc;
        scattered = scatter<true>(S, m, ray, rec, g, k, att, sc, tex, 0.0, marble);
        if (scattered) {
            if (!marble) T = T * att;
            ray = sc;
            depth -= 1u;
            done = depth == 0u;
        } else {
            done = true;
        }
    }
    PROF_T0(pmw);
    const double turb = turbulence_wave(S.perm, marble, mp, tab);
    PROF_ADD(kPrMarble, pmw);
    if (marble) {
        const float sv = 0.5f * (1.0f + rt_sinf(mscale * mp.z + 10.0f * (float)turb));
        if (mlight) L = L + T * mk(sv, sv, sv);
        else if (scattered) T = T * mk(sv, sv, sv);
    }
    if (shade && done) {
        sbuf_store<kF>(sbuf + ((size_t)s_local * Q.nslots + slot) * 3u, L);
    }
    return shade && done;
}

#ifndef RT_SUSPEND
#define RT_SUSPEND 24
#endif
constexpr uint32_t kSuspLanes = RT_SUSPEND;
template <int kKind, int kWaves = 3, uint32_t kF = kFAll>
__global__ __launch_bounds__(64, kWaves) void trace_samples(DevScene Sg, DevCamera C, DevParams P, ChunkParams Q,
                                                    float* __restrict__ sbuf, TraceCounters* __restrict__ ctr,
                                                    ReplayItem* __restrict__ replay_list, uint32_t fixup,
                                                    unsigned long long* __restrict__ seg_counter) {
    extern __shared__ uint32_t lds_stack[];
    const uint32_t lane = threadIdx.x;
    uint32_t* stk = lds_stack + lane;
    DevScene S = Sg;
    if (S.perm_bytes != 0u && S.perm_bytes <= kPermLdsMax && !(P.tune & kModeNoPermLds)) {
        uint32_t* tab = lds_stack + S.stack_depth * 128u;
        const uint32_t* src = reinterpret_cast<const uint32_t*>(Sg.perm);
        for (uint32_t i = lane; i < S.perm_bytes / 4u; i += 64u) tab[i] = src[i];
        __syncthreads();
        S.perm = reinterpret_cast<const uint8_t*>(tab);
    }
    if constexpr (kKind == 0 && (kF & (kFBvh | kFTri | kFMarble)) == 0u) {
        if (S.mt_lds) {
            uint32_t* tab = lds_stack + S.stack_depth * 128u;
            const uint32_t nm = S.num_mats * (sizeof(DevMaterial) / 4u), nt = S.num_texs * (sizeof(DevTexture) / 4u);
            const uint32_t* sm = reinterpret_cast<const uint32_t*>(Sg.mats);
            const uint32_t* st = reinterpret_cast<const uint32_t*>(Sg.texs);
            for (uint32_t i = lane; i < nm; i += 64u) tab[i] = sm[i];
            for (uint32_t i = lane; i < nt; i += 64u) tab[nm + i] = st[i];
            __syncthreads();
            S.mats = reinterpret_cast<const DevMaterial*>(tab);
            S.texs = reinterpret_cast<const DevTexture*>(tab + nm);
        }
    }
    if (kKind == 2) {
        const uint32_t perm_words =
            S.perm_bytes != 0u && S.perm_bytes <= kPermLdsMax && !(P.tune & kModeNoPermLds) ? S.perm_bytes / 4u : 0u;
        S.hrpp_cnt = lds_stack + S.stack_depth * 128u + perm_words;
        if (lane < 4u * S.hrpp_npred) S.hrpp_cnt[lane] = 0u;
        __syncthreads();
    }
    const Key k{P.seed_lo, P.seed_hi};
    const uint32_t mode = P.tune;
#ifdef RT_CAMMEM
    const DevCamera& Cs = *reinterpret_cast<const DevCamera*>(reinterpret_cast<const char*>(ctr) + kCamOffset);
#else
    const DevCamera& Cs = C;
#endif
    unsigned* counter = &ctr->batch;
    const ReplayItem* list = nullptr;
    uint32_t list_n = 0u, stream_grid = 0u;
    if ((kKind == 1 || kKind == 3) && fixup == 2u) {
        if (__hip_atomic_load(&ctr->batch, __ATOMIC_RELAXED, __HIP_MEMORY_SCOPE_AGENT) < Q.units) return;
        list = replay_list;
        list_n = kReplayCap;
        counter = &ctr->replay_pull;
        stream_grid = Q.fast_grid;
    } else if ((kKind == 1 || kKind == 3) && fixup) {
        const uint32_t n = __hip_atomic_load(&ctr->replay_count, __ATOMIC_RELAXED, __HIP_MEMORY_SCOPE_AGENT);
        const bool abort = __hip_atomic_load(&ctr->stream_abort, __ATOMIC_RELAXED, __HIP_MEMORY_SCOPE_AGENT) != 0u;
        if (n <= kReplayCap && !abort) {
            if (n == 0u) return;
            list = replay_list;
            list_n = n;
            counter = &ctr->replay_pull;
        } else {
            counter = &ctr->batch_full;
            for (uint32_t i = blockIdx.x * 64u + lane; i < kReplayCap; i += gridDim.x * 64u)
                (void)replay_take(replay_list, i);
            if (blockIdx.x == 0u && lane == 0u && seg_counter)
                atomicAdd(seg_counter, 0ull - __hip_atomic_load(&ctr->fast_segments, __ATOMIC_RELAXED,
                                                                __HIP_MEMORY_SCOPE_AGENT));
        }
    }
    bool has = false;
    uint32_t slot = 0, take_sample_idx = 0, depth = 0;
    uint32_t nseg = 0;
    V L = mk(0.0f, 0.0f, 0.0f), T = mk(1.0f, 1.0f, 1.0f);
    Rng g{};
    Ray ray{};
    ItemPool pool{0u, 0u, 0u, false};
    PROF_INIT();
#ifdef RT_PROFILE_REGIONS
    const unsigned long long wave_t0 = __builtin_amdgcn_s_memrealtime();
    uint32_t tp_bucket = 0u, tp_acc = 0u;
#endif
    if constexpr (kKind == 0 && (kF & kFSusp) != 0u) {
        Walk w{};
        w.pos = 0u;
        for (;;) {
            PROF_T0(pr);
            if (take_sample(pool, !has, Cs, P, Q, k, counter, list, list_n, ctr, stream_grid, sbuf, lane, slot, take_sample_idx, L, T, depth, g,
                            ray)) {
                has = true;
                w.pos = 0u;
                w.resume = false;
            }
            PROF_ADD(kPrRefill, pr);
            if (__ballot(has) == 0ull) break;
            if (has && w.pos == 0u && !w.resume) {
                w.closest = kInf;
                w.any = false;
            }
            bool replay = false;
            PROF_T0(pw);
            world_walk<kF>(S, P.prune_delta, ray, g, k, w, has, stk, mode, replay, pool.exhausted ? 0u : kSuspLanes);
            PROF_ADD(kPrWorld, pw);
            if (has && replay) {
                unsigned idx = atomicAdd(&ctr->replay_count, 1u);
                if (idx < kReplayCap) replay_publish(replay_list, idx, g.pixel, g.sample - Q.sample0);
                has = false;
            }
            const bool walked = has && w.pos == S.num_top;
            if constexpr ((kF & kFMarble) != 0u) {
                if (shade_marble<kF>(S, P, Q, k, sbuf, walked, w.any, w.hit_entry, w.hit_code, w.closest, ray, L, T,
                                     depth, g, slot, g.sample - Q.sample0)) {
                    has = false;
                    nseg += P.max_depth - depth + (depth != 0u ? 1u : 0u);
                }
            } else if (walked && finish_segment<kF>(S, P, Q, k, sbuf, w.any, w.hit_entry, w.hit_code, w.closest, ray, L,
                                                    T, depth, g, slot, g.sample - Q.sample0)) {
                has = false;
                nseg += P.max_depth - depth + (depth != 0u ? 1u : 0u);
            }
            if (walked) w.pos = 0u;
        }
    } else
    for (;;) {
        PROF_T0(pr);
        if (take_sample(pool, !has, Cs, P, Q, k, counter, list, list_n, ctr, stream_grid, sbuf, lane, slot, take_sample_idx, L, T, depth, g,
                        ray)) {
            has = true;
        }
        PROF_ADD(kPrRefill, pr);
        if (__ballot(has) == 0ull) break;
#ifdef RT_PROFILE_REGIONS
        if (kKind == 0) {
            const uint32_t b = (uint32_t)((__builtin_amdgcn_s_memrealtime() - wave_t0) / kTpTicks);
            if (b != tp_bucket) {
                if (lane == 0u && tp_acc && tp_bucket < kTpBuckets) atomicAdd(&g_tp_hist[tp_bucket], tp_acc);
                tp_bucket = b;
                tp_acc = 0u;
            }
            tp_acc += (uint32_t)__popcll(__ballot(has));
        }
#endif
        if constexpr ((kF & kFMarble) != 0u) {
            bool shade = false, any = false;
            float t = 0.0f;
            uint32_t he = 0, hc = 0;
            if (has) {
                bool replay = false;
                PROF_T0(pw);
                any = world_hit<kKind, kF>(S, P.prune_delta, ray, g, k, t, he, hc, stk, mode, replay);
                PROF_ADD(kPrWorld, pw);
                if (kKind == 0 && replay) {
                    unsigned idx = atomicAdd(&ctr->replay_count, 1u);
                    if (idx < kReplayCap) replay_publish(replay_list, idx, g.pixel, g.sample - Q.sample0);
                    has = false;
                } else {
                    shade = true;
                }
            }
            if (shade_marble<kF>(S, P, Q, k, sbuf, shade, any, he, hc, t, ray, L, T, depth, g, slot, g.sample - Q.sample0)) {
                has = false;
                nseg += P.max_depth - depth + (depth != 0u ? 1u : 0u);
            }
        } else if (has) {
            float t;
            uint32_t he = 0, hc = 0;
            bool replay = false;
            PROF_T0(pw);
            bool any = world_hit<kKind, kF>(S, P.prune_delta, ray, g, k, t, he, hc, stk, mode, replay);
            PROF_ADD(kPrWorld, pw);
            if (kKind == 0 && replay) {
                unsigned idx = atomicAdd(&ctr->replay_count, 1u);
                if (idx < kReplayCap) replay_publish(replay_list, idx, g.pixel, g.sample - Q.sample0);
                has = false;
            } else if (finish_segment<kF>(S, P, Q, k, sbuf, any, he, hc, t, ray, L, T, depth, g, slot, g.sample - Q.sample0)) {
                has = false;
                nseg += P.max_depth - depth + (depth != 0u ? 1u : 0u);
            }
        }
    }
    if (kKind == 2) {
        __syncthreads();
        if (lane < 4u * S.hrpp_npred) atomicAdd(&S.hrpp_stats[lane], (unsigned long long)S.hrpp_cnt[lane]);
    }
    if (seg_counter) {
        unsigned long long v = (unsigned long long)nseg;
        for (int off = 32; off > 0; off >>= 1) v += __shfl_xor(v, off);
        if (lane == 0u) {
            atomicAdd(seg_counter, v);
            if (kKind == 0 || stream_grid) atomicAdd(&ctr->fast_segments, v);
        }
    }
    if (kKind == 0 && lane == 0u) {
        __threadfence();
        atomicAdd(&ctr->fast_done, 1u);
    }
    PROF_FLUSH();
#ifdef RT_PROFILE_REGIONS
    if (kKind == 0 && lane == 0u && tp_acc && tp_bucket < kTpBuckets) atomicAdd(&g_tp_hist[tp_bucket], tp_acc);
    if (stream_grid && lane == 0u) role_event(0xfffffffeu);
    if (kKind == 0 && lane == 0u && blockIdx.x < kProfWaves) {
        g_wave_t[2u * blockIdx.x] = wave_t0;
        g_wave_t[2u * blockIdx.x + 1u] = __builtin_amdgcn_s_memrealtime();
    }
#endif
}

__global__ __launch_bounds__(256) void resolve_samples(const float* __restrict__ sbuf, float* __restrict__ out,
                                                        DevParams P, ChunkParams Q, int first, int last) {
    const uint32_t t = blockIdx.x * 256u + threadIdx.x;
    if (t >= Q.nslots) return;
    const uint32_t blk = P.shard_index + (t >> 6) * P.shard_count, pib = t & 63u;
    const uint32_t by = blk / P.blocks_x, bx = blk - by * P.blocks_x;
    const uint32_t x = bx * 8u + (pib & 7u), y = by * 8u + (pib >> 3);
    if (x >= P.width || y >= P.height) return;
    float* o = out + ((size_t)y * P.width + x) * 3u;
    V acc = first ? mk(0.0f, 0.0f, 0.0f) : mk(o[0], o[1], o[2]);
    const float* src = sbuf + (size_t)t * 3u;
    const size_t plane = (size_t)Q.nslots * 3u;
    for (uint32_t s = 0; s < Q.samples; ++s) {
        acc = acc + mk(src[0], src[1], src[2]);
        src += plane;
    }
    if (last) acc = divs(acc, (float)P.spp_div);
    o[0] = acc.x;
    o[1] = acc.y;
    o[2] = acc.z;
}

__global__ void numeric_eval(int op, const double* a, const double* b, double* out, uint32_t n) {
    uint32_t i = blockIdx.x * blockDim.x + threadIdx.x;
    if (i >= n) return;
    double x = a[i], y = b ? b[i] : 0.0;
    double r = 0.0;
    switch (op) {
        case 0: r = __builtin_sqrt(x); break;
        case 1: r = (double)__builtin_sqrtf((float)x); break;
        case 2: r = (double)((float)x / (float)y); break;
        case 3: r = (double)rt_sinf((float)x); break;
        case 4: r = (double)rt_acosf((float)x); break;
        case 5: r = (double)rt_atan2f((float)x, (float)y); break;
        case 6: r = (double)rt_logf((float)x); break;
        case 7: r = x / y; break;
        case 8: r = (double)hrpp_map_float((float)x); break;
        default: r = 0.0; break;
    }
    out[i] = r;
}

__global__ void kat_eval(int op, const float* __restrict__ in, float* __restrict__ out, uint32_t n) {
    uint32_t i = blockIdx.x * blockDim.x + threadIdx.x;
    if (i >= n) return;
    float r0 = 0.0f, r1 = 0.0f;
    if (op == 0 || op == 1) {
        const float* a = in + 14u * i;
        Ray r;
        r.o = mk(a[6], a[7], a[8]);
        r.d = mk(a[9], a[10], a[11]);
        r.time = 0.0f;
        const V inv = mk(1.0f / r.d.x, 1.0f / r.d.y, 1.0f / r.d.z);
        if (op == 0) {
            float te = 0.0f;
            r0 = slab(a[0], a[1], a[2], a[3], a[4], a[5], r, inv, a[12], a[13], te) ? 1.0f : 0.0f;
            r1 = te;
        } else {
            const float E = kInf;
            f4 mnx{a[0], E, E, E}, mny{a[1], E, E, E}, mnz{a[2], E, E, E};
            f4 mxx{a[3], -E, -E, -E}, mxy{a[4], -E, -E, -E}, mxz{a[5], -E, -E, -E};
            float key[4];
            child_keys4_nf(inv.x < 0.0f ? mxx : mnx, inv.y < 0.0f ? mxy : mny, inv.z < 0.0f ? mxz : mnz,
                           inv.x < 0.0f ? mnx : mxx, inv.y < 0.0f ? mny : mxy, inv.z < 0.0f ? mnz : mxz, r, inv,
                           a[12], a[13], kInf, 0.0f, key);
            r0 = key[0] != kInf ? 1.0f : 0.0f;
            r1 = key[0];
        }
    } else if (op == 2) {
        const float* a = in + 3u * i;
        sphere_uv(mk(a[0], a[1], a[2]), r0, r1);
    } else if (op == 4) {
        const float kk = in[3u * i], o = in[3u * i + 1u], d = in[3u * i + 2u];
        const auto zero = [](float v) { return (__float_as_uint(v) & 0x7fffffffu) == 0u; };
        const bool gate = (__float_as_uint(kk) == 0u || rcp_range(kk)) && (zero(o) || rcp_range(o)) && rcp_range(d);
        r0 = gate ? rcp_quotient(kk, o, d, 1.0f / d) : (kk - o) / d;
        r1 = (kk - o) / d;
    } else if (op == 3) {
        const float* a = in + 12u * i;
        Ray r;
        r.o = mk(a[4], a[5], a[6]);
        r.d = mk(a[7], a[8], a[9]);
        r.time = 0.0f;
        float t = 0.0f;
        r0 = sphere_t(f4{a[0], a[1], a[2], a[3]}, to_d(r), a[10], a[11], t) ? 1.0f : 0.0f;
        r1 = t;
    }
    out[2u * i] = r0;
    out[2u * i + 1u] = r1;
}

}

#if defined(RT_INSTANCES_TU) && RT_INSTANCES_TU == 1
void* rt_mc_trace_instance(uint32_t preset) {
    if (preset == kFBvh) return reinterpret_cast<void*>(trace_samples<0, 4, kFBvh>);
    if (preset == (kFBvh | kFMarble)) return reinterpret_cast<void*>(trace_samples<0, 4, kFBvh | kFMarble>);
    if (preset == kFRuns) return reinterpret_cast<void*>(trace_samples<0, 4, kFRuns>);
    return nullptr;
}
#elif defined(RT_INSTANCES_TU) && RT_INSTANCES_TU == 2
void* rt_flat_trace_instance(int waves) {
    return waves == 4 ? reinterpret_cast<void*>(trace_samples<0, 4, 0u>) : reinterpret_cast<void*>(trace_samples<0, 3, 0u>);
}
#else
#ifdef RT_SPLIT_MC
void* rt_mc_trace_instance(uint32_t preset);
void* rt_flat_trace_instance(int waves);
#endif

namespace {
__global__ __launch_bounds__(256) void hrpp_count(const rtdev::HrppSlot* __restrict__ tab, uint32_t bits, uint32_t np,
                                                  unsigned long long* __restrict__ out) {
    const uint64_t per = 1ull << bits;
    for (uint32_t p = 0; p < np; ++p) {
        unsigned long long keys = 0, ids = 0;
        for (uint64_t i = blockIdx.x * 256ull + threadIdx.x; i < per; i += (uint64_t)gridDim.x * 256u) {
            const rtdev::HrppSlot& sl = tab[(uint64_t)p * per + i];
            if (sl.key == ~0ull) continue;
            keys += 1;
            for (uint32_t j = 0; j < rtdev::kHrppIds; ++j) ids += sl.ids[j] != 0xffffffffu ? 1u : 0u;
        }
        for (int off = 32; off > 0; off >>= 1) {
            keys += __shfl_xor(keys, off);
            ids += __shfl_xor(ids, off);
        }
        if ((threadIdx.x & 63u) == 0u) {
            atomicAdd(&out[2 * p], keys);
            atomicAdd(&out[2 * p + 1], ids);
        }
    }
}
__global__ void store_camera(DevCamera c, DevCamera* __restrict__ dst) {
    constexpr uint32_t kWords = sizeof(DevCamera) / sizeof(uint32_t);
    static_assert(sizeof(DevCamera) % sizeof(uint32_t) == 0, "DevCamera is whole words");
    const uint32_t i = threadIdx.x;
    if (i < kWords) {
        uint32_t w;
        __builtin_memcpy(&w, reinterpret_cast<const char*>(&c) + 4u * i, 4u);
        reinterpret_cast<uint32_t*>(dst)[i] = w;
    }
}
}

struct rt_scene {
    int device = 0;
    void* pool = nullptr;
    uint64_t pool_bytes = 0;
    DevScene dev{};
    uint64_t counts[10] = {};
    float* sbuf = nullptr;
    uint64_t sbuf_bytes = 0;
    TraceCounters* counter = nullptr;
    uint32_t stack_ref = 1;
    int grid = 0, grid_ref = 0;
    int fast_waves = 0;
    uint32_t features = kFAll;
    uint32_t* stack_spill = nullptr;
    ReplayItem* replay = nullptr;
    hipStream_t aux = nullptr;
    hipEvent_t fork = nullptr, join = nullptr;
    float coord_bound = 0.0f;
    rtdev::HrppSlot* hrpp_tab = nullptr;
    uint64_t hrpp_tab_bytes = 0;
    uint32_t hrpp_bits = 0;
    unsigned long long* hrpp_stats = nullptr;
    static constexpr int kEvents = 256;
    hipEvent_t ev[kEvents][2] = {};
    int ev_count = 0;
    bool ev_overflow = false;
    std::mutex mu;
    hipEvent_t done = nullptr;
};

namespace {

int hip_fail(hipError_t e, const char* what) {
    return rthost::set_error(RT_ERR_HIP, std::string(what) + ": " + hipGetErrorString(e));
}

struct DeviceGuard {
    int prev = -1;
    bool ok = false;
    explicit DeviceGuard(int dev) {
        if (hipGetDevice(&prev) != hipSuccess) prev = -1;
        ok = hipSetDevice(dev) == hipSuccess;
    }
    ~DeviceGuard() {
        if (prev >= 0) (void)hipSetDevice(prev);
    }
};

using TraceKernel = void (*)(DevScene, DevCamera, DevParams, ChunkParams, float*, TraceCounters*, ReplayItem*, uint32_t,
                             unsigned long long*);
template <int kWaves, uint32_t kF>
TraceKernel preset_instance() {
#ifdef RT_SPLIT_MC
    if constexpr (kWaves == 4 && (kF == kFBvh || kF == (kFBvh | kFMarble) || kF == kFRuns))
        return reinterpret_cast<TraceKernel>(rt_mc_trace_instance(kF));
    else if constexpr (kF == 0u)
        return reinterpret_cast<TraceKernel>(rt_flat_trace_instance(kWaves));
    else
#endif
        return trace_samples<0, kWaves, kF>;
}
template <int kWaves>
TraceKernel fast_instance(uint32_t features) {
    switch (preset_of(features)) {
        case 0u: return preset_instance<kWaves, 0u>();
        case kFRuns: return preset_instance<kWaves, kFRuns>();
        case kFBvh: return preset_instance<kWaves, kFBvh>();
        case kFBvh | kFMarble: return preset_instance<kWaves, kFBvh | kFMarble>();
        case kFBvh | kFTri | kFDeep | kFSusp:
            return preset_instance<kWaves, kFBvh | kFTri | kFDeep | kFSusp>();
        default: return preset_instance<kWaves, kFAll>();
    }
}
TraceKernel fast_instance(int waves, uint32_t features) {
    return waves == 4 ? fast_instance<4>(features) : fast_instance<3>(features);
}

std::atomic<int64_t> g_opt[RT_OPT_COUNT] = {{0}, {0}, {0}, {0}, {-1}, {0}, {0}, {0}, {0}};
int64_t opt(int o) { return g_opt[o].load(std::memory_order_relaxed); }

int check_device(int device) {
    int n = 0;
    hipError_t e = hipGetDeviceCount(&n);
    if (e != hipSuccess || n == 0)
        return rthost::set_error(RT_ERR_NO_DEVICE, "no HIP device visible (the device path has no CPU fallback)");
    if (device < 0 || device >= n) return rthost::set_error(RT_ERR_INVALID, "device index out of range");
    hipDeviceProp_t prop;
    if (hipGetDeviceProperties(&prop, device) != hipSuccess) return rthost::set_error(RT_ERR_NO_DEVICE, "device query failed");
    if (strncmp(prop.gcnArchName, "gfx950", 6) != 0)
        return rthost::set_error(RT_ERR_NO_DEVICE, std::string("device is ") + prop.gcnArchName +
                                                       "; this build targets gfx950 (MI355X) only");
    return RT_OK;
}

int check_params(const rt_render_params* p) {
    if (!p) return rthost::set_error(RT_ERR_INVALID, "params is NULL");
    if (p->width == 0 || p->height == 0) return rthost::set_error(RT_ERR_INVALID, "empty image");
    if (p->samples_per_pixel == 0) return rthost::set_error(RT_ERR_INVALID, "samples_per_pixel must be > 0");
// ... 36 lines not shown
    if (hs.num_predictors > rtdev::kHrppMaxPredictors)
        return rthost::set_error(RT_ERR_UNSUPPORTED, "more than 8 Bvh::with_predictor BVHs");
    struct Part {
        const void* src;
        uint64_t bytes;
        uint64_t off;
    };
    std::vector<Part> parts = {
        {hs.entries.data(), hs.entries.size() * sizeof(DevEntry), 0},
        {hs.sph.data(), hs.sph.size() * sizeof(f4), 0},
        {hs.sph_mat.data(), hs.sph_mat.size() * sizeof(uint32_t), 0},
        {hs.msph.data(), hs.msph.size() * sizeof(f4), 0},
        {hs.rect.data(), hs.rect.size() * sizeof(f4), 0},
        {hs.tri.data(), hs.tri.size() * sizeof(f4), 0},
        {hs.nodes.data(), hs.nodes.size() * sizeof(f4), 0},
        {hs.mats.data(), hs.mats.size() * sizeof(DevMaterial), 0},
        {hs.texs.data(), hs.texs.size() * sizeof(DevTexture), 0},
        {hs.perm.data(), hs.perm.size(), 0},
        {hs.texels.data(), hs.texels.size(), 0},
        {hs.nodes2.data(), hs.nodes2.size() * sizeof(f4), 0},
        {hs.hrpp_keys.data(), hs.hrpp_keys.size() * sizeof(uint64_t), 0},
        {hs.hrpp_vals.data(), hs.hrpp_vals.size() * sizeof(uint32_t), 0},
    };
    uint64_t total = 0;
    for (auto& p : parts) {
        p.off = total;
        total += (p.bytes + 255u) & ~255ull;
    }
    if (total == 0) total = 256;
    rt_scene* s = new (std::nothrow) rt_scene();
    if (!s) return rthost::set_error(RT_ERR_OOM, "host allocation failed");
    s->device = device;
    {
        DeviceGuard g(device);
        hipError_t e = hipMalloc(&s->pool, total);
        if (e != hipSuccess) {
            delete s;
            return rthost::set_error(RT_ERR_OOM, std::string("hipMalloc scene: ") + hipGetErrorString(e));
        }
        std::vector<uint8_t> staging(total, 0);
        for (auto& p : parts)
            if (p.bytes) memcpy(staging.data() + p.off, p.src, p.bytes);
        e = hipMemcpy(s->pool, staging.data(), total, hipMemcpyHostToDevice);
        if (e != hipSuccess) {
            (void)hipFree(s->pool);
            delete s;
            return hip_fail(e, "hipMemcpy scene");
        }
    }
    uint8_t* base = (uint8_t*)s->pool;
    s->pool_bytes = total;
    DevScene& d = s->dev;
    d.entries = (const DevEntry*)(base + parts[0].off);
    d.sph = (const f4*)(base + parts[1].off);
    d.sph_mat = (const uint32_t*)(base + parts[2].off);
    d.msph = (const f4*)(base + parts[3].off);
    d.rect = (const f4*)(base + parts[4].off);
    d.tri = (const f4*)(base + parts[5].off);
    d.nodes = (const f4*)(base + parts[6].off);
    d.mats = (const DevMaterial*)(base + parts[7].off);
    d.texs = (const DevTexture*)(base + parts[8].off);
    d.num_mats = (uint32_t)hs.mats.size();
    d.num_texs = (uint32_t)hs.texs.size();
    d.mt_lds = 0u;
    d.perm = base + parts[9].off;
    d.texels = base + parts[10].off;
    d.nodes2 = (const f4*)(base + parts[11].off);
    d.num_nodes = (uint32_t)(hs.nodes.size() / rtdev::kBvhNodeF4);
    d.num_nodes2 = (uint32_t)(hs.nodes2.size() / 4);
    d.num_top = hs.num_top;
    d.num_entries = (uint32_t)hs.entries.size();
    d.stack_depth = hs.max_stack;
#ifdef RT_LEAF_AUDIT
    d.stack_depth = std::max(hs.max_stack, hs.max_stack_ref);
#endif
    s->stack_ref = hs.max_stack_ref;
    d.perm_bytes = (uint32_t)hs.perm.size();
    d.hrpp_tab = nullptr;
    d.hrpp_keys = (const unsigned long long*)(base + parts[12].off);
    d.hrpp_vals = (const uint32_t*)(base + parts[13].off);
    d.hrpp_nkeys = (uint32_t)hs.hrpp_keys.size();
    d.hrpp_npred = hs.num_predictors;
    s->coord_bound = hs.coord_bound;
    d.rect_rcp_ok = 1u;
    for (size_t i = 0; i + 1 < hs.rect.size(); i += 2) {
        const rtdev::f4 r0 = hs.rect[i], r1 = hs.rect[i + 1];
        for (float c : {r0.x, r0.y, r0.z, r0.w, r1.x}) {
            uint32_t b;
            memcpy(&b, &c, 4);
            const float a = std::fabs(c);
            if (!(b == 0u || (a >= 0x1p-20f && a <= 0x1p20f))) d.rect_rcp_ok = 0u;
        }
    }
    d.mb_entry = ~0u;
    for (uint32_t e = 0; e < hs.num_top; ++e) {
        const rtdev::DevEntry& E = hs.entries[e];
        if (E.kind == rtdev::kEntMedium) {
            const rtdev::DevEntry& B = hs.entries[E.payload];
            if (B.kind == rtdev::kEntGeom && rtdev::leaf_type(B.payload) == rtdev::kLeafSphere) d.mb_entry = e;
            break;
        }
        bool ok = E.kind == rtdev::kEntSphereRun || E.kind == rtdev::kEntRectRun;
        if (E.kind == rtdev::kEntGeom) ok = rtdev::leaf_type(E.payload) != rtdev::kLeafTri;
        if (E.kind == rtdev::kEntBvh) {
            uint32_t flag;
            memcpy(&flag, &hs.nodes[(size_t)E.payload * rtdev::kBvhNodeF4 + 7].w, 4);
            ok = (flag & rtdev::kBvhPrunable) != 0u;
            for (uint32_t i = 0; i < E.ntf && i < (uint32_t)rtdev::kMaxTransforms; ++i) ok = ok && E.tf[i].w == 0.0f;
        }
        if (!ok) break;
    }
    s->features = (hs.tri.empty() ? 0u : kFTri) | (hs.bvh_rect_msph ? kFLeafRM : 0u);
    for (const rtdev::DevTexture& t : hs.texs)
        if (t.kind == rtdev::kTexMarble) s->features |= kFMarble;
#ifndef RT_LEAF_AUDIT
    {
        uint32_t cap = kStackLdsMax;
        if (const int64_t v = opt(RT_OPT_STACK_LDS))
            cap = std::min(cap, (uint32_t)v);
        if (hs.max_stack > cap) {
            s->features |= kFDeep;
            d.stack_depth = cap;
            d.spill_depth = hs.max_stack - cap;
        }
    }
#endif
    for (const rtdev::DevEntry& e : hs.entries) {
        if (e.kind == rtdev::kEntBvh) s->features |= kFBvh;
        if (e.kind == rtdev::kEntSphereRun && e.pad[0] >= kRunPretestMin) s->features |= kFRuns;
    }
    uint64_t c[10] = {hs.entries.size(), hs.sph.size(), hs.msph.size() / 3, hs.rect.size() / 2, hs.tri.size() / 3,
                      hs.nodes.size() / rtdev::kBvhNodeF4, hs.mats.size(), hs.texs.size(), hs.max_bvh_depth, total};
    memcpy(s->counts, c, sizeof c);
    *out = s;
    return RT_OK;
}

int rt_scene_free(rt_scene_handle s) {
    rthost::clear_error();
    if (!s) return RT_OK;
    {
        DeviceGuard g(s->device);
#ifdef RT_PROFILE_REGIONS
        static unsigned long long hc[kProfCopies * kProfWords];
        unsigned long long h[kProfWords] = {};
        if (hipDeviceSynchronize() == hipSuccess && hipMemcpyFromSymbol(hc, HIP_SYMBOL(g_prof), sizeof hc) == hipSuccess) {
            for (uint32_t c = 0; c < kProfCopies; ++c)
                for (uint32_t i = 0; i < kProfWords; ++i) h[i] += hc[c * kProfWords + i];
            fprintf(stderr, "{\"rt_profile\": [");
            for (uint32_t i = 0; i < 3u * kPrCount; ++i) fprintf(stderr, "%s%llu", i ? "," : "", h[i]);
            fprintf(stderr, "]}\n");
        }
        {
            const unsigned long long* th = h + 3u * kPrCount;
            fprintf(stderr, "{\"trips_hist\": [%llu,%llu,%llu,%llu,%llu,%llu,%llu,%llu], \"wave_max_hist\": "
                            "[%llu,%llu,%llu,%llu,%llu,%llu,%llu,%llu]}\n",
                    th[0], th[1], th[2], th[3], th[4], th[5], th[6], th[7], th[8], th[9], th[10], th[11], th[12],
                    th[13], th[14], th[15]);
        }
        {
            static unsigned long long wt[2 * kProfWaves];
            if (hipMemcpyFromSymbol(wt, HIP_SYMBOL(g_wave_t), sizeof wt) == hipSuccess) {
                std::vector<unsigned long long> st, en;
                for (uint32_t i = 0; i < kProfWaves; ++i)
                    if (wt[2 * i + 1]) {
                        st.push_back(wt[2 * i]);
                        en.push_back(wt[2 * i + 1]);
                    }
                if (!st.empty()) {
                    std::sort(st.begin(), st.end());
                    std::sort(en.begin(), en.end());
                    const unsigned long long t0 = st.front();
                    auto q = [&](const std::vector<unsigned long long>& v, double f) {
                        return (double)(v[(size_t)(f * (double)(v.size() - 1))] - t0) / 100.0;
                    };
                    fprintf(stderr, "{\"wave_times_us\": {\"waves\": %zu, \"start\": [%.1f, %.1f, %.1f], "
                                    "\"end\": [%.1f, %.1f, %.1f, %.1f, %.1f]}}\n",
                            st.size(), q(st, 0.5), q(st, 0.99), q(st, 1.0), q(en, 0.0), q(en, 0.1), q(en, 0.5),
                            q(en, 0.9), q(en, 1.0));
                }
            }
            static unsigned long long rv[2 * kRoleEvents];
            unsigned rn = 0;
            if (hipMemcpyFromSymbol(&rn, HIP_SYMBOL(g_role_n), sizeof rn) == hipSuccess && rn &&
                hipMemcpyFromSymbol(rv, HIP_SYMBOL(g_role_ev), sizeof rv) == hipSuccess) {
                unsigned long long t0 = ~0ull;
                for (uint32_t i = 0; i < kProfWaves; ++i)
                    if (wt[2 * i + 1] && wt[2 * i] < t0) t0 = wt[2 * i];
                fprintf(stderr, "{\"role_events_us\": [");
                for (unsigned i = 0; i < rn && i < kRoleEvents; ++i)
                    fprintf(stderr, "%s[%.1f, %lld]", i ? "," : "", ((double)rv[2 * i] - (double)t0) / 100.0,
                            rv[2 * i + 1] >= 0xfffffffeull ? -(long long)(rv[2 * i + 1] - 0xfffffffdull) : (long long)rv[2 * i + 1]);
                fprintf(stderr, "]}\n");
            }
            static unsigned long long tp[kTpBuckets];
            if (hipMemcpyFromSymbol(tp, HIP_SYMBOL(g_tp_hist), sizeof tp) == hipSuccess) {
                uint32_t n = kTpBuckets;
                while (n > 0u && tp[n - 1u] == 0u) --n;
                fprintf(stderr, "{\"tp_gseg_per_s\": {\"bucket_us\": %u, \"rate\": [", kTpTicks / 100u);
                for (uint32_t i = 0; i < n; ++i)
                    fprintf(stderr, "%s%.3f", i ? "," : "", (double)tp[i] / (kTpTicks * 10.0));
                fprintf(stderr, "]}}\n");
            }
        }
#endif
#ifdef RT_DEBUG_PIXEL
        {
            unsigned nd = 0;
            static uint32_t dv[8 * kDbgMax];
            if (hipMemcpyFromSymbol(&nd, HIP_SYMBOL(g_dbg_n), sizeof nd) == hipSuccess &&
                hipMemcpyFromSymbol(dv, HIP_SYMBOL(g_dbg), sizeof dv) == hipSuccess)
                for (unsigned i = 0; i < nd && i < kDbgMax; ++i)
                    fprintf(stderr, "DBG %u %08x %08x %08x %08x %08x %08x %08x\n", dv[8 * i], dv[8 * i + 1],
                            dv[8 * i + 2], dv[8 * i + 3], dv[8 * i + 4], dv[8 * i + 5], dv[8 * i + 6], dv[8 * i + 7]);
        }
#endif
#ifdef RT_LEAF_AUDIT
        unsigned na = 0;
        static LeafAudit au[kAuditMax];
        if (hipMemcpyFromSymbol(&na, HIP_SYMBOL(g_audit_count), sizeof na) == hipSuccess &&
            hipMemcpyFromSymbol(au, HIP_SYMBOL(g_audit), sizeof au) == hipSuccess) {
            fprintf(stderr, "{\"leaf_audit_count\": %u}\n", na);
            for (unsigned i = 0; i < na && i < kAuditMax; ++i)
                fprintf(stderr,
                        "{\"audit\": {\"o\": [%a, %a, %a], \"d\": [%a, %a, %a], \"tmin\": %a, \"closest\": %a, "
                        "\"t\": %a, \"box\": [%a, %a, %a, %a, %a, %a], \"delta\": %a, \"code\": %u, \"rank\": %u, "
                        "\"best_rank\": %u}}\n",
                        au[i].o[0], au[i].o[1], au[i].o[2], au[i].d[0], au[i].d[1], au[i].d[2], au[i].tmin,
                        au[i].closest, au[i].t, au[i].box[0], au[i].box[1], au[i].box[2], au[i].box[3], au[i].box[4],
                        au[i].box[5], au[i].delta, au[i].code, au[i].rank, au[i].best_rank);
        }
        static TravAudit ta[kAuditMax];
        if (hipMemcpyFromSymbol(&na, HIP_SYMBOL(g_trav_audit_count), sizeof na) == hipSuccess &&
            hipMemcpyFromSymbol(ta, HIP_SYMBOL(g_trav_audit), sizeof ta) == hipSuccess) {
            fprintf(stderr, "{\"trav_audit_count\": %u}\n", na);
            for (unsigned i = 0; i < na && i < kAuditMax; ++i)
                fprintf(stderr,
                        "{\"trav_audit\": {\"o\": [%a, %a, %a], \"d\": [%a, %a, %a], \"tmin\": %a, \"tmax\": %a, "
                        "\"fast_t\": %a, \"ref_t\": %a, \"fast_code\": %u, \"ref_code\": %u, \"root\": %u}}\n",
                        ta[i].o[0], ta[i].o[1], ta[i].o[2], ta[i].d[0], ta[i].d[1], ta[i].d[2], ta[i].tmin, ta[i].tmax,
                        ta[i].fast_t, ta[i].ref_t, ta[i].fast_code, ta[i].ref_code, ta[i].root);
        }
        if (hipMemcpyFromSymbol(&na, HIP_SYMBOL(g_bounds_audit_count), sizeof na) == hipSuccess)
            fprintf(stderr, "{\"bounds_audit_count\": %u}\n", na);
#endif
        if (s->done) (void)hipEventSynchronize(s->done);
        if (s->pool) (void)hipFree(s->pool);
        if (s->sbuf) (void)hipFree(s->sbuf);
        if (s->counter) (void)hipFree(s->counter);
        if (s->stack_spill) (void)hipFree(s->stack_spill);
        if (s->replay) (void)hipFree(s->replay);
        if (s->fork) (void)hipEventDestroy(s->fork);
        if (s->join) (void)hipEventDestroy(s->join);
        if (s->aux) (void)hipStreamDestroy(s->aux);
        if (s->hrpp_tab) (void)hipFree(s->hrpp_tab);
        if (s->hrpp_stats) (void)hipFree(s->hrpp_stats);
        for (int i = 0; i < rt_scene::kEvents; ++i)
            for (int j = 0; j < 2; ++j)
                if (s->ev[i][j]) (void)hipEventDestroy(s->ev[i][j]);
        if (s->done) (void)hipEventDestroy(s->done);
    }
    delete s;
    return RT_OK;
}

int rt_scene_hrpp_stats(rt_scene_handle s, uint64_t* out, uint32_t capacity, uint32_t* count) {
    rthost::clear_error();
    if (!s || !count) return rthost::set_error(RT_ERR_INVALID, "NULL argument");
    const uint32_t np = s->dev.hrpp_npred;
    *count = np;
    if (!out || capacity < 6u * np) return capacity == 0 ? RT_OK : rthost::set_error(RT_ERR_INVALID, "capacity < 6 per predictor");
    memset(out, 0, sizeof(uint64_t) * 6u * np);
    if (!s->hrpp_stats) return RT_OK;
    DeviceGuard g(s->device);
    unsigned long long h[4 * rtdev::kHrppMaxPredictors] = {};
    unsigned long long* d_tab_counts = nullptr;
    hipError_t e;
    if ((e = hipMalloc(&d_tab_counts, 16u * np)) != hipSuccess ||
        (e = hipMemset(d_tab_counts, 0, 16u * np)) != hipSuccess) {
        if (d_tab_counts) (void)hipFree(d_tab_counts);
        return hip_fail(e, "HRPP stats");
    }
    (void)hipGetLastError();
    if (s->hrpp_bits)
        hipLaunchKernelGGL(hrpp_count, dim3(1024), dim3(256), 0, nullptr, s->hrpp_tab, s->hrpp_bits, np, d_tab_counts);
    unsigned long long tc[2 * rtdev::kHrppMaxPredictors] = {};
    if ((e = hipGetLastError()) != hipSuccess || (e = hipDeviceSynchronize()) != hipSuccess ||
        (e = hipMemcpy(h, s->hrpp_stats, 32u * np, hipMemcpyDeviceToHost)) != hipSuccess ||
        (e = hipMemcpy(tc, d_tab_counts, 16u * np, hipMemcpyDeviceToHost)) != hipSuccess) {
        (void)hipFree(d_tab_counts);
        return hip_fail(e, "HRPP stats");
    }
    (void)hipFree(d_tab_counts);
    for (uint32_t p = 0; p < np; ++p) {
        out[6 * p + 0] = h[4 * p + 0];
        out[6 * p + 1] = h[4 * p + 1];
        out[6 * p + 2] = h[4 * p + 2];
        out[6 * p + 3] = tc[2 * p + 0];
        out[6 * p + 4] = tc[2 * p + 1];
        out[6 * p + 5] = h[4 * p + 3];
    }
    return RT_OK;
}

int rt_scene_info(rt_scene_handle s, uint64_t counts[10]) {
    rthost::clear_error();
    if (!s || !counts) return rthost::set_error(RT_ERR_INVALID, "NULL argument");
    memcpy(counts, s->counts, sizeof s->counts);
    return RT_OK;
}

int rt_camera_new(const rt_camera_desc* args, rt_camera* out) {
    rthost::clear_error();
    if (!args || !out) return rthost::set_error(RT_ERR_INVALID, "NULL argument");
    std::string err;
    int rc = rthost::camera_new(args, out, &err);
    return rc ? rthost::set_error(rc, err) : RT_OK;
}

int rt_render_launch(rt_scene_handle s, const rt_camera_desc* camera, const rt_render_params* p, float* d_out,
                     unsigned long long* d_segments, void* stream) {
    rthost::clear_error();
    if (!camera) return rthost::set_error(RT_ERR_INVALID, "NULL camera");
    rt_camera cam;
    std::string err;
    int rc = rthost::camera_new(camera, &cam, &err);
    if (rc) return rthost::set_error(rc, err);
    return rt_render_launch_camera(s, &cam, p, d_out, d_segments, stream);
}

int rt_render_launch_camera(rt_scene_handle s, const rt_camera* camera, const rt_render_params* p, float* d_out,
                            unsigned long long* d_segments, void* stream) {
    rthost::clear_error();
    if (!s || !camera || !d_out) return rthost::set_error(RT_ERR_INVALID, "NULL scene/camera/output");
    int rc = check_params(p);
    if (rc) return rc;
    DevCamera cam;
    std::string err;
    if ((rc = rthost::camera_device(camera, &cam, &err))) return rthost::set_error(rc, err);
    DevParams dp;
    memset(&dp, 0, sizeof dp);
    dp.width = p->width;
    dp.height = p->height;
    dp.spp = p->samples_per_pixel;
    dp.max_depth = p->max_depth;
    dp.seed_lo = (uint32_t)p->seed;
    dp.seed_hi = (uint32_t)(p->seed >> 32);
    dp.sample_base = p->sample_base;
    dp.shard_count = p->shard_count > 1 ? p->shard_count : 1u;
    dp.shard_index = p->shard_count > 1 ? p->shard_index : 0u;
    dp.blocks_x = (p->width + 7u) / 8u;
    dp.num_blocks = dp.blocks_x * ((p->height + 7u) / 8u);
    dp.flags = p->flags;
    dp.spp_div = p->spp_total ? p->spp_total : p->samples_per_pixel;
    dp.tune = (uint32_t)opt(RT_OPT_TUNE) & ~kModeExact;
    dp.bg[0] = p->background[0];
    dp.bg[1] = p->background[1];
    dp.bg[2] = p->background[2];
    {
        double R = sqrt((double)cam.origin[0] * cam.origin[0] + (double)cam.origin[1] * cam.origin[1] +
                        (double)cam.origin[2] * cam.origin[2]) +
                   2.0 * (double)fabsf(cam.lens_radius) + 2.0 * (double)s->coord_bound;
        double delta = R * (1.0 / 1048576.0) * 1.01 + 1e-30;
        dp.prune_delta = (float)delta;
        if (!(dp.prune_delta < 1e30f)) dp.flags |= RT_FLAG_EXACT_BVH;
    }
    uint32_t nblk = dp.num_blocks > dp.shard_index ? (dp.num_blocks - dp.shard_index + dp.shard_count - 1u) / dp.shard_count : 0u;
#ifdef RT_PROFILE_REGIONS
    if (g_prof_rows[1] != 0xffffffffu && dp.shard_count == 1u) {
        const uint32_t rows = (dp.height + 7u) / 8u;
        const uint32_t r0 = std::min(g_prof_rows[0], rows), r1 = std::min(std::max(g_prof_rows[1], r0), rows);
        dp.shard_index = r0 * dp.blocks_x;
        nblk = (r1 - r0) * dp.blocks_x;
    }
#endif
    if (nblk == 0) return RT_OK;
    DeviceGuard g(s->device);
    if (!g.ok) return rthost::set_error(RT_ERR_HIP, "hipSetDevice failed");
    std::lock_guard<std::mutex> lock(s->mu);
    hipError_t e;
    if (!s->done && (e = hipEventCreateWithFlags(&s->done, hipEventDisableTiming)) != hipSuccess) {
        s->done = nullptr;
        return hip_fail(e, "hipEventCreate");
    }
    if ((e = hipStreamWaitEvent((hipStream_t)stream, s->done, 0)) != hipSuccess) return hip_fail(e, "hipStreamWaitEvent");
    const uint64_t nslots = (uint64_t)nblk * 64u;
    const uint64_t per_sample = nslots * 3u * sizeof(float);
    uint64_t budget = 8192ull << 20;
    {
        size_t free_b = 0, total_b = 0;
        if (s->sbuf_bytes >= per_sample * p->samples_per_pixel) {
            budget = s->sbuf_bytes;
        } else if (hipMemGetInfo(&free_b, &total_b) == hipSuccess) {
            const uint64_t avail = (uint64_t)((double)(free_b + s->sbuf_bytes) * 0.4);
            if (avail > budget) budget = avail;
        }
    }
// ... 289 lines not shown
    int rc = check_params(p);
    if (rc) return rc;
    if (p->shard_count > 1) return rthost::set_error(RT_ERR_INVALID, "rt_render_multi shards the frame itself");
    for (uint32_t i = 0; i < n; ++i)
        if (!scenes[i]) return rthost::set_error(RT_ERR_INVALID, "NULL scene handle");
    const size_t floats = (size_t)p->width * p->height * 3u;
    struct Shard {
        int device = 0;
        hipStream_t st = nullptr;
        hipEvent_t e0 = nullptr, e1 = nullptr;
        float* d_out = nullptr;
        unsigned long long* d_seg = nullptr;
        unsigned long long seg = 0;
        std::vector<float> img;
    };
    std::vector<Shard> sh(n);
    auto cleanup = [&]() {
        for (Shard& x : sh) {
            DeviceGuard g(x.device);
            if (x.st) (void)hipStreamSynchronize(x.st);
            if (x.e0) (void)hipEventDestroy(x.e0);
            if (x.e1) (void)hipEventDestroy(x.e1);
            if (x.st) (void)hipStreamDestroy(x.st);
            if (x.d_out) (void)hipFree(x.d_out);
            if (x.d_seg) (void)hipFree(x.d_seg);
        }
    };
    hipError_t e;
    for (uint32_t i = 0; i < n; ++i) {
        Shard& x = sh[i];
        x.device = scenes[i]->device;
        DeviceGuard g(x.device);
        if (!g.ok) { cleanup(); return rthost::set_error(RT_ERR_HIP, "hipSetDevice failed"); }
        if ((e = hipStreamCreateWithFlags(&x.st, hipStreamNonBlocking)) != hipSuccess) { cleanup(); return hip_fail(e, "hipStreamCreate"); }
        if ((e = hipMalloc(&x.d_out, floats * sizeof(float))) != hipSuccess ||
            (e = hipMalloc(&x.d_seg, sizeof(unsigned long long))) != hipSuccess) {
            cleanup();
            return rthost::set_error(RT_ERR_OOM, "hipMalloc shard image");
        }
        if (((p->flags & RT_FLAG_ACCUMULATE)
                 ? (e = hipMemcpyAsync(x.d_out, host_out, floats * sizeof(float), hipMemcpyHostToDevice, x.st))
                 : (e = hipMemsetAsync(x.d_out, 0, floats * sizeof(float), x.st))) != hipSuccess ||
            (e = hipMemsetAsync(x.d_seg, 0, sizeof(unsigned long long), x.st)) != hipSuccess) {
            cleanup();
            return hip_fail(e, "shard image init");
        }
        (void)hipEventCreate(&x.e0);
        (void)hipEventCreate(&x.e1);
        (void)hipEventRecord(x.e0, x.st);
        rt_render_params q = *p;
        q.shard_index = n > 1 ? i : 0u;
        q.shard_count = n > 1 ? n : 0u;
        if ((rc = rt_render_launch_camera(scenes[i], camera, &q, x.d_out, x.d_seg, x.st))) { cleanup(); return rc; }
        (void)hipEventRecord(x.e1, x.st);
        x.img.resize(floats);
        if ((e = hipMemcpyAsync(x.img.data(), x.d_out, floats * sizeof(float), hipMemcpyDeviceToHost, x.st)) != hipSuccess ||
            (e = hipMemcpyAsync(&x.seg, x.d_seg, sizeof x.seg, hipMemcpyDeviceToHost, x.st)) != hipSuccess) {
            cleanup();
            return hip_fail(e, "D2H shard");
        }
    }
    float ms_max = 0.0f;
    for (Shard& x : sh) {
        DeviceGuard g(x.device);
        if ((e = hipStreamSynchronize(x.st)) != hipSuccess) { cleanup(); return hip_fail(e, "render shard"); }
        float ms = 0.0f;
        (void)hipEventElapsedTime(&ms, x.e0, x.e1);
        ms_max = ms > ms_max ? ms : ms_max;
    }
    const uint32_t bxn = (p->width + 7u) / 8u;
    unsigned long long seg = 0;
    for (uint32_t y = 0; y < p->height; ++y)
        for (uint32_t x = 0; x < p->width; ++x) {
            const uint32_t owner = ((y / 8u) * bxn + x / 8u) % n;
            const size_t o = ((size_t)y * p->width + x) * 3u;
            memcpy(host_out + o, sh[owner].img.data() + o, 3u * sizeof(float));
        }
    for (Shard& x : sh) seg += x.seg;
    if (stats) {
        stats->segments = seg;
        stats->samples = (uint64_t)p->width * p->height * p->samples_per_pixel;
        stats->kernel_ms = ms_max;
    }
    cleanup();
    return RT_OK;
}

int rt_set_option(int option, int64_t value) {
    rthost::clear_error();
    if (option < 0 || option >= RT_OPT_COUNT) return rthost::set_error(RT_ERR_INVALID, "unknown option");
    bool ok = true;
    switch (option) {
        case RT_OPT_TUNE:
            ok = value >= 0 && value <= 0xffffffffll && ((uint64_t)value & ~(uint64_t)kTuneAccepted) == 0u;
            break;
        case RT_OPT_GROUP: ok = value >= 0 && value <= 64; break;
        case RT_OPT_STACK_LDS: ok = value >= 0 && value <= 96; break;
        case RT_OPT_SAMPLE_BUFFER_MB: ok = value >= 0 && value <= (1ll << 30); break;
        case RT_OPT_HRPP_SLOT_BITS: ok = value >= -1 && value <= 28; break;
        case RT_OPT_LAUNCH_LOG: ok = value == 0 || value == 1; break;
        case RT_OPT_BVH_BUILD: ok = value >= 0 && value <= 2; break;
        case RT_OPT_GUIDE: ok = value >= 0 && value <= 256; break;
        case RT_OPT_BVH_SHAPE: ok = value == 0 || value == 1; break;
    }
    if (!ok) return rthost::set_error(RT_ERR_INVALID, "option value out of range");
    g_opt[option].store(value, std::memory_order_relaxed);
    return RT_OK;
}

int rt_get_option(int option, int64_t* value) {
    rthost::clear_error();
    if (option < 0 || option >= RT_OPT_COUNT || !value) return rthost::set_error(RT_ERR_INVALID, "unknown option");
    *value = opt(option);
    return RT_OK;
}

int rt_scene_trace_time(rt_scene_handle s, double* total_ms, uint64_t* launches, int reset) {
    rthost::clear_error();
    if (!s || !total_ms || !launches) return rthost::set_error(RT_ERR_INVALID, "NULL argument");
    DeviceGuard g(s->device);
    std::lock_guard<std::mutex> lock(s->mu);
    double sum = 0.0;
    for (int i = 0; i < s->ev_count; ++i) {
        hipError_t e = hipEventSynchronize(s->ev[i][1]);
        if (e != hipSuccess) return hip_fail(e, "hipEventSynchronize");
        float ms = 0.0f;
        if ((e = hipEventElapsedTime(&ms, s->ev[i][0], s->ev[i][1])) != hipSuccess) return hip_fail(e, "hipEventElapsedTime");
        sum += ms;
    }
    *total_ms = sum;
    *launches = (uint64_t)s->ev_count;
    if (s->ev_overflow) {
        if (reset) {
            s->ev_count = 0;
            s->ev_overflow = false;
        }
        return rthost::set_error(RT_ERR_INVALID, "more than 256 launches since the last reset: timing incomplete");
    }
    if (reset) s->ev_count = 0;
    return RT_OK;
}

#ifdef RT_PROFILE_REGIONS
int rt_prof_rows(uint32_t r0, uint32_t r1) {
    g_prof_rows[0] = r0;
    g_prof_rows[1] = r1;
    return RT_OK;
}
#endif

int rt_device_kat(int op, const float* in, float* out, uint32_t n) {
    rthost::clear_error();
    if (!in || !out) return rthost::set_error(RT_ERR_INVALID, "NULL argument");
    if (op < 0 || op > 4) return rthost::set_error(RT_ERR_INVALID, "unknown KAT op");
    int rc = check_device(0);
    if (rc) return rc;
    if (n == 0) return RT_OK;
    DeviceGuard g(0);
    const size_t in_floats = (size_t)n * (op <= 1 ? 14u : (op == 2 || op == 4 ? 3u : 12u)),
                 out_floats = (size_t)n * 2u;
    float *din = nullptr, *dout = nullptr;
    hipError_t e = hipMalloc(&din, in_floats * sizeof(float));
    if (e == hipSuccess) e = hipMalloc(&dout, out_floats * sizeof(float));
    if (e == hipSuccess) e = hipMemcpy(din, in, in_floats * sizeof(float), hipMemcpyHostToDevice);
    if (e == hipSuccess) {
        (void)hipGetLastError();
        hipLaunchKernelGGL(kat_eval, dim3((n + 63u) / 64u), dim3(64), 0, nullptr, op, din, dout, n);
        e = hipGetLastError();
    }
    if (e == hipSuccess) e = hipMemcpy(out, dout, out_floats * sizeof(float), hipMemcpyDeviceToHost);
    if (din) (void)hipFree(din);
    if (dout) (void)hipFree(dout);
    if (e != hipSuccess) return hip_fail(e, "kat_eval");
    return RT_OK;
}

int rt_device_numeric_eval(int op, const double* a, const double* b, double* out, uint32_t n) {
    rthost::clear_error();
    if (!a || !out) return rthost::set_error(RT_ERR_INVALID, "NULL argument");
    int rc = check_device(0);
    if (rc) return rc;
    if (n == 0) return RT_OK;
    DeviceGuard g(0);
    double *da = nullptr, *db = nullptr, *dout = nullptr;
    size_t bytes = (size_t)n * sizeof(double);
    hipError_t e = hipMalloc(&da, bytes);
    if (e == hipSuccess && b) e = hipMalloc(&db, bytes);
    if (e == hipSuccess) e = hipMalloc(&dout, bytes);
    if (e == hipSuccess) e = hipMemcpy(da, a, bytes, hipMemcpyHostToDevice);
    if (e == hipSuccess && b) e = hipMemcpy(db, b, bytes, hipMemcpyHostToDevice);
    if (e == hipSuccess) {
        (void)hipGetLastError();
        hipLaunchKernelGGL(numeric_eval, dim3((n + 255u) / 256u), dim3(256), 0, nullptr, op, da, db, dout, n);
        e = hipGetLastError();
    }
    if (e == hipSuccess) e = hipMemcpy(out, dout, bytes, hipMemcpyDeviceToHost);
    if (da) (void)hipFree(da);
    if (db) (void)hipFree(db);
    if (dout) (void)hipFree(dout);
    if (e != hipSuccess) return hip_fail(e, "numeric_eval");
    return RT_OK;
}

}
#endif
```

Baseline: 1282 Msamples/s.

## Add quad-cooperative BVH tail traversal for divergent wave remainders

```diff
diff --git a/raytracinginoneweekendinrust_amd/__init__.py b/raytracinginoneweekendinrust_amd/__init__.py
--- a/raytracinginoneweekendinrust_amd/__init__.py
+++ b/raytracinginoneweekendinrust_amd/__init__.py
@@ -512,6 +512,15 @@
     return out
 
 
+def device_kat_quad(cases) -> np.ndarray:
+    a = np.ascontiguousarray(cases, dtype=np.float32)
+    assert a.ndim == 2 and a.shape[1] == 40, a.shape
+    out = np.zeros((a.shape[0], 24), dtype=np.float32)
+    check(lib.rt_device_kat(5, a.ctypes.data_as(C.POINTER(C.c_float)), out.ctypes.data_as(C.POINTER(C.c_float)),
+                            a.shape[0]), "rt_device_kat")
+    return out.view(np.uint32)
+
+
 def numeric_eval(op: int, a: np.ndarray, b: Optional[np.ndarray] = None) -> np.ndarray:
     a = np.ascontiguousarray(a, dtype=np.float64)
     out = np.empty_like(a)
diff --git a/raytracinginoneweekendinrust_amd/csrc/kernel.hip b/raytracinginoneweekendinrust_amd/csrc/kernel.hip
--- a/raytracinginoneweekendinrust_amd/csrc/kernel.hip
+++ b/raytracinginoneweekendinrust_amd/csrc/kernel.hip
@@ -35,7 +35,7 @@
     kPrRefill = 0, kPrSegment, kPrWorld, kPrRecord, kPrEmit, kPrScatter, kPrMarble, kPrStore,
     kPrChecker, kPrImage, kPrUnitSphere, kPrDielectric, kPrLambert, kPrMetal, kPrIso, kPrLog,
     kPrEntry0 = 16, kPrEntryLast = 43, kPrBvhTrip = 44, kPrLeafTest = 45, kPrBvhSetup = 46, kPrBvhPush = 47,
-    kPrBvhPop = 48, kPrBvhCall = 49, kPrCount = 52
+    kPrBvhPop = 48, kPrBvhCall = 49, kPrQuadIter = 50, kPrQuadRepack = 51, kPrCount = 52
 };
 constexpr uint32_t kModeExact = 1u, kModeNoLeafBoxes = 2u, kModeNoPermLds = 32u, kModeW3 = 64u,
                    kModeNoPretest = 128u, kModeReplayRef = 1u << 16;
@@ -48,9 +48,10 @@
 #endif
 constexpr uint32_t kModeBlocksForward = 1u << 21;
 constexpr uint32_t kModeW4 = 1u << 22;
+constexpr uint32_t kModeQuadShift = 13u, kModeQuadMask = 7u << kModeQuadShift;
 [[maybe_unused]] constexpr uint32_t kModeMbShrink = 1u << 29;
 constexpr uint32_t kTuneExact = kModeNoLeafBoxes | kModeNoPermLds | kModeW3 | kModeNoPretest | kModeReplayRef |
-                                kModeNoStream | kModeBlocksForward | kModeW4 | (15u << 24);
+                                kModeNoStream | kModeBlocksForward | kModeW4 | (15u << 24) | kModeQuadMask;
 constexpr uint32_t kTuneAccepted = kTuneExact
 #if defined(RT_LEAF_AUDIT) || defined(RT_ABLATE)
                                    | kModePruneAllExp
@@ -74,7 +75,10 @@
 #endif
 #ifdef RT_PROFILE_REGIONS
 constexpr uint32_t kProfCopies = 64;
-constexpr uint32_t kProfWords = 3 * kPrCount + 16;
+constexpr uint32_t kLiveClasses = 9, kLiveBins = 28, kLiveRows = 5;
+constexpr uint32_t kLiveWords = kLiveClasses * kLiveRows * kLiveBins;
+constexpr uint32_t kProfLive0 = 3 * kPrCount + 16, kProfScratch0 = kProfLive0 + kLiveWords;
+constexpr uint32_t kProfWords = kProfScratch0 + 3;
 __device__ unsigned long long g_prof[kProfCopies * kProfWords];
 constexpr uint32_t kProfWaves = 8192;
 __device__ unsigned long long g_wave_t[2 * kProfWaves];
@@ -100,7 +104,7 @@
 }
 __device__ __forceinline__ void prof_flush() {
     unsigned long long* dst = g_prof + (blockIdx.x % kProfCopies) * kProfWords;
-    for (uint32_t i = threadIdx.x; i < kProfWords; i += blockDim.x)
+    for (uint32_t i = threadIdx.x; i < kProfScratch0; i += blockDim.x)
         if (prof_lds[i]) atomicAdd(&dst[i], prof_lds[i]);
 }
 #define PROF_T0(name) const uint64_t name = __builtin_amdgcn_s_memtime()
@@ -114,13 +118,44 @@
         prof_lds[2 * kPrCount + region] += (uint64_t)__popcll(m);
     }
 }
+__device__ __forceinline__ uint32_t live_bin(uint32_t n) { return n <= 16u ? n - 1u : 16u + (n - 17u) / 4u; }
+__device__ __forceinline__ unsigned long long* live_row(uint32_t row) {
+    const uint32_t cls = (uint32_t)prof_lds[kProfScratch0];
+    return prof_lds + kProfLive0 + ((cls < kLiveClasses ? cls : kLiveClasses - 1u) * kLiveRows + row) * kLiveBins;
+}
+__device__ __forceinline__ void prof_set_entry(uint32_t e) {
+    if (__lane_id() == (uint32_t)__builtin_ctzll(__ballot(1))) prof_lds[kProfScratch0] = e;
+}
+__device__ __forceinline__ void prof_live_iter(uint32_t row, uint32_t n) {
+    const uint64_t now = __builtin_amdgcn_s_memtime();
+    if (__lane_id() == (uint32_t)__builtin_ctzll(__ballot(1))) {
+        const uint32_t open = (uint32_t)prof_lds[kProfScratch0 + 2u];
+        if (open) {
+            unsigned long long* h = live_row(row);
+            h[open - 1u] += now - prof_lds[kProfScratch0 + 1u];
+            h[kLiveBins + open - 1u] += 1u;
+        }
+        prof_lds[kProfScratch0 + 1u] = now;
+        prof_lds[kProfScratch0 + 2u] = n ? live_bin(n) + 1u : 0u;
+    }
+}
+__device__ __forceinline__ void prof_live_call() {
+    const uint64_t m = __ballot(1);
+    if (__lane_id() == (uint32_t)__builtin_ctzll(m)) live_row(4u)[live_bin((uint32_t)__popcll(m))] += 1u;
+}
 #define PROF_INIT() prof_init()
 #define PROF_FLUSH() prof_flush()
+#define PROF_ENTRY(e) prof_set_entry(e)
+#define PROF_LIVE_ITER(row, n) prof_live_iter((row), (n))
+#define PROF_LIVE_CALL() prof_live_call()
 #else
 #define PROF_T0(name) do { } while (0)
 #define PROF_ADD(region, t0) do { } while (0)
 #define PROF_INIT() do { } while (0)
 #define PROF_FLUSH() do { } while (0)
+#define PROF_ENTRY(e) do { } while (0)
+#define PROF_LIVE_ITER(row, n) do { } while (0)
+#define PROF_LIVE_CALL() do { } while (0)
 #endif
 #ifdef RT_LEAF_AUDIT
 struct LeafAudit {
@@ -973,9 +1008,22 @@
 #define RT_LEAF_Q 8
 #endif
 
-template <int kKind, uint32_t kF, bool kSusp>
+template <int kKind, uint32_t kF, bool kSusp, uint32_t kMinTrips = kSuspMinTrips>
 RT_DEV bool bvh_run(const DevScene& S, float delta, const f4* wrapper, const Ray& r, V inv, float tmin, float& closest,
                     uint32_t& hit_code, uint32_t* stk, uint32_t mode, Trav& tv, uint32_t susp);
+#ifndef RT_QUAD_TAIL
+#define RT_QUAD_TAIL 1
+#endif
+#if defined(RT_SPLIT_MC) && !defined(RT_INSTANCES_TU)
+constexpr bool kQuadTailUnit = false;
+#else
+constexpr bool kQuadTailUnit = RT_QUAD_TAIL;
+#endif
+template <int kKind, uint32_t kF>
+constexpr bool kQuadTail = kQuadTailUnit && kKind == 0 && kF == (kFBvh | kFMarble);
+template <uint32_t kF>
+RT_DEV void bvh_quad_tail(const DevScene& S, float delta, const f4* wrapper, const Ray& r, V inv, float tmin,
+                          float& closest, uint32_t& hit_code, uint32_t* stk, uint32_t mode, Trav& tv, bool live);
 constexpr uint32_t kRayFast = 0u, kRayHandOver = 1u, kRayNoHit = 2u;
 #ifndef RT_TRI_ZERO_DIR_FAST
 #define RT_TRI_ZERO_DIR_FAST 1
@@ -1040,7 +1088,7 @@
 #define RT_PEEL_WRAPPER 1
 #endif
 constexpr bool kPeelWrapper = RT_PEEL_WRAPPER;
-template <int kKind, uint32_t kF = kFAll>
+template <int kKind, uint32_t kF = kFAll, bool kTopWalk = false>
 RT_DEV bool bvh_hit(const DevScene& S, float delta, uint32_t root, const Ray& r, float tmin, float& closest,
                     uint32_t& hit_code, uint32_t* stk, uint32_t mode, bool& replay) {
     PROF_T0(pcall);
@@ -1080,6 +1128,7 @@
         }
     }
     PROF_ADD(kPrBvhSetup, psetup);
+    PROF_LIVE_CALL();
     Trav tv{root, 0u, 0u, closest, false, kNoNode};
     if constexpr (kPeelWrapper) {
         const f4 w0 = ld4c(wrapper), w1 = ld4c(wrapper + 1), w2 = ld4c(wrapper + 2), w3 = ld4c(wrapper + 3),
@@ -1094,7 +1143,20 @@
         const float lo = __builtin_fmaxf(__builtin_fmaxf(tnx, tny), __builtin_fmaxf(tnz, tmin));
         const float hi = __builtin_fminf(__builtin_fminf(tfx, tfy), __builtin_fminf(tfz, closest));
         const float te = lo - (prune ? dmi : 0.0f);
-        if (lo <= hi && te <= (prune ? prune_bound(closest) : kInf)) {
+        if constexpr (kQuadTail<kKind, kF> && kTopWalk) {
+            const uint32_t tq = (mode >> kModeQuadShift) & 7u;
+            const uint64_t m = __ballot(1);
+            const uint32_t nhost = (uint32_t)__popcll(m & (m >> 1) & (m >> 2) & (m >> 3) & 0x1111111111111111ull);
+            const uint32_t cap = tq == 0u ? 16u : 2u * tq;
+            const uint32_t lim = tq == 1u ? 0u : (nhost < cap ? nhost : cap);
+            bool live = false;
+            if (lo <= hi && te <= (prune ? prune_bound(closest) : kInf)) {
+                tv.cur = __float_as_uint(w6.x);
+                live = !bvh_run<kKind, kF, true, 0u>(S, delta, wrapper, r, inv, tmin, closest, hit_code, stk, mode, tv, lim);
+            }
+            if (__ballot(live) != 0ull)
+                bvh_quad_tail<kF>(S, delta, wrapper, r, inv, tmin, closest, hit_code, stk, mode, tv, live);
+        } else if (lo <= hi && te <= (prune ? prune_bound(closest) : kInf)) {
             tv.cur = __float_as_uint(w6.x);
             bvh_run<kKind, kF, false>(S, delta, wrapper, r, inv, tmin, closest, hit_code, stk, mode, tv, 0u);
         }
@@ -1107,12 +1169,13 @@
     return any;
 }
 
-#ifndef RT_POP_PREFETCH
-#define RT_POP_PREFETCH 0
-#endif
 template <uint32_t kF>
-constexpr bool kPopPrefetch = RT_POP_PREFETCH && (kF & (kFTri | kFDeep)) == 0u;
-template <int kKind, uint32_t kF, bool kSusp>
+RT_DEV void leaf_node_visit(const DevScene& S, float delta, uint32_t lnode, uint32_t onx, uint32_t ony, uint32_t onz,
+                            bool leaf_boxes, float tmax_entry, const Ray& r, V inv, float tmin, float& closest,
+                            uint32_t& best_rank, uint32_t& hit_code, bool& any, [[maybe_unused]] uint32_t mode) {
+#include "leaf_node_body.inc"
+}
+template <int kKind, uint32_t kF, bool kSusp, uint32_t kMinTrips>
 RT_DEV bool bvh_run(const DevScene& S, float delta, const f4* wrapper, const Ray& r, V inv, float tmin, float& closest,
                     uint32_t& hit_code, uint32_t* stk, uint32_t mode, Trav& tv, uint32_t susp) {
     const float tmax_entry = tv.tmax_entry;
@@ -1134,12 +1197,13 @@
 #endif
     for (;;) {
         if constexpr (kSusp) {
-            if (trips >= kSuspMinTrips && (uint32_t)__popcll(__ballot(1)) <= susp) {
+            if (trips >= kMinTrips && (uint32_t)__popcll(__ballot(1)) <= susp) {
                 finished = false;
                 break;
             }
             ++trips;
         }
+        PROF_LIVE_ITER(0u, (uint32_t)__popcll(__ballot(1)));
         uint32_t lnode = kNoNode;
         bool popnext = false, do_int;
         if constexpr (kPostpone) {
@@ -1195,88 +1259,13 @@
 #ifdef RT_PROFILE_REGIONS
         ++visits;
 #endif
-        [[maybe_unused]] uint32_t pf_node = 0u;
-        [[maybe_unused]] float pf_t = 0.0f;
-        if constexpr (kPopPrefetch<kF>) {
-            const uint32_t top = (sp > 0u ? sp - 1u : 0u) * 128u;
-            pf_node = stk[top];
-            pf_t = __uint_as_float(stk[top + 64u]);
-        }
         PROF_T0(pt);
         if (lnode != kNoNode) {
-            const uint32_t nbo = (lnode & ~rtdev::kLeafNodeFlag) * (rtdev::kBvhNodeF4 * 16u);
-            const f4* nd = S.nodes;
-            const float2 nx2 = ld2_at(nd, nbo + onx), ny2 = ld2_at(nd, nbo + ony), nz2 = ld2_at(nd, nbo + onz),
-                         fx2 = ld2_at(nd, nbo + (onx ^ 48u)), fy2 = ld2_at(nd, nbo + (ony ^ 80u)),
-                         fz2 = ld2_at(nd, nbo + (onz ^ 112u)), chs = ld2_at(nd, nbo + 96u), rks = ld2_at(nd, nbo + 112u);
-            float tmr = tmax_entry, nt = 0.0f;
-            bool nh = false;
-            uint32_t ncode = 0u, nrank = 0u;
-            const uint32_t nleaf = __float_as_uint(chs.y) == rtdev::kChildEmpty ? 1u : 2u;
-            float llo[2] = {-kInf, -kInf}, lhi[2] = {kInf, kInf};
-            if (leaf_boxes) leaf_intervals2_nf(nx2, ny2, nz2, fx2, fy2, fz2, r, inv, delta, llo, lhi);
-            for (uint32_t k = 0; k < nleaf; ++k) {
-                const uint32_t lcode = __float_as_uint(k ? chs.y : chs.x), rank = __float_as_uint(k ? rks.y : rks.x);
-#ifdef RT_LEAF_AUDIT
-                const float2 bx0 = ld2(S.nodes + nbo / 16u, 0), by0 = ld2(S.nodes + nbo / 16u, 1),
-                             bz0 = ld2(S.nodes + nbo / 16u, 2), bx1 = ld2(S.nodes + nbo / 16u, 3),
-                             by1 = ld2(S.nodes + nbo / 16u, 4), bz1 = ld2(S.nodes + nbo / 16u, 5);
-                const float x0 = k ? bx0.y : bx0.x, y0 = k ? by0.y : by0.x, z0 = k ? bz0.y : bz0.x;
-                const float x1 = k ? bx1.y : bx1.x, y1 = k ? by1.y : by1.x, z1 = k ? bz1.y : bz1.x;
-#endif
-                const float bound = tmr < closest ? tmr : closest;
-                if (!leaf_boxes || leaf_interval_may_hit(k ? llo[1] : llo[0], k ? lhi[1] : lhi[0], tmin, bound)) {
-                    PROF_T0(pl);
-                    const float cap = closest < kInf ? __uint_as_float(__float_as_uint(closest) + 1u) : kInf;
-                    float c = tmr < cap ? tmr : cap;
-                    uint32_t code = 0u;
-                    const RayD q = to_d(r);
-                    ABLATE(kAbLeaf2, float c2 = c; uint32_t h2 = 0u;
-                           if (leaf_hit<kF>(S, lcode, r, q, tmin, c2, h2) && h2 == 0x7fffffffu) c = -1.0f;);
-                    bool hit;
-                    if constexpr (kLeafEmbed<kF>) {
-                        const uint32_t ltype = rtdev::leaf_type(lcode);
-                        const uint32_t lo = nbo + 4u * k;
-                        if (ltype == rtdev::kLeafSphere) {
-                            const f4 sp{ld1_at(nd, lo + 8u), ld1_at(nd, lo + 24u), ld1_at(nd, lo + 40u), ld1_at(nd, lo + 104u)};
-                            float ts;
-                            hit = sphere_t(sp, q, tmin, c, ts);
-                            if (hit) {
-                                c = ts;
-                                code = lcode;
-                            }
-                        } else if (ltype == rtdev::kLeafCube) {
-                            hit = cube_hit<(kF & kFTri) == 0u>(S, rtdev::leaf_index(lcode), ld1_at(nd, lo), ld1_at(nd, lo + 16u),
-                                                               ld1_at(nd, lo + 32u), ld1_at(nd, lo + 48u), ld1_at(nd, lo + 64u),
-                                                               ld1_at(nd, lo + 80u), r, inv, tmin, c, code);
-                        } else {
-                            hit = leaf_hit<kF, (kF & kFTri) == 0u, false, true>(S, lcode, r, q, tmin, c, code, inv);
-                        }
-                    } else {
-                        hit = leaf_hit<kF, (kF & kFTri) == 0u>(S, lcode, r, q, tmin, c, code, inv);
-                    }
-                    if (hit) {
-                        const uint32_t rk = rank + (rtdev::leaf_type(lcode) == rtdev::kLeafCube
-                                                        ? rtdev::leaf_index(code) - rtdev::leaf_index(lcode)
-                                                        : 0u);
-                        if (!nh || !(nt < c)) {
-                            nh = true;
-                            nt = c;
-                            ncode = code;
-                            nrank = rk;
-                        }
-                        tmr = c;
-                    }
-                    PROF_ADD(kPrLeafTest, pl);
-                } else {
-                    LEAF_AUDIT(lcode, rank, x0, y0, z0, x1, y1, z1);
-                }
-            }
-            if (nh && (nt < closest || (nt == closest && nrank > best_rank))) {
-                closest = nt;
-                best_rank = nrank;
-                hit_code = ncode;
-                any = true;
+            if constexpr (kQuadTail<kKind, kF>) {
+                leaf_node_visit<kF>(S, delta, lnode, onx, ony, onz, leaf_boxes, tmax_entry, r, inv, tmin, closest,
+                                    best_rank, hit_code, any, mode);
+            } else {
+#include "leaf_node_body.inc"
             }
         }
         float t0 = kInf, t1 = kInf, t2 = kInf, t3 = kInf;
@@ -1346,16 +1335,11 @@
         PROF_T0(ppop);
         if (popnext) {
             bool found = false;
-            [[maybe_unused]] bool first = true;
             while (sp > 0u) {
                 sp -= 1u;
                 uint32_t cand;
                 float tenter;
-                if (kPopPrefetch<kF> && first) {
-                    cand = pf_node;
-                    tenter = pf_t;
-                    first = false;
-                } else if (!(kF & kFDeep) || sp < S.stack_depth) {
+                if (!(kF & kFDeep) || sp < S.stack_depth) {
                     cand = stk[sp * 128u];
                     tenter = __uint_as_float(stk[sp * 128u + 64u]);
                 } else {
@@ -1385,6 +1369,7 @@
         }
     }
     tv = Trav{cur, sp, best_rank, tmax_entry, any, pend};
+    PROF_LIVE_ITER(0u, 0u);
 #ifdef RT_PROFILE_REGIONS
     {
         const uint32_t b = trips_bin(visits);
@@ -1402,6 +1387,172 @@
     }
 #endif
     return finished;
+}
+
+constexpr int kQuadRot1 = 0x39, kQuadRot2 = 0x4e, kQuadRot3 = 0x93, kQuadLane0 = 0x00, kQuadXor1 = 0xb1;
+template <int kCtrl>
+RT_DEV uint32_t quad_perm(uint32_t v) {
+    return (uint32_t)__builtin_amdgcn_update_dpp(0, (int)v, kCtrl, 0xf, 0xf, false);
+}
+template <int kCtrl>
+RT_DEV float quad_perm(float v) {
+    return __uint_as_float(quad_perm<kCtrl>(__float_as_uint(v)));
+}
+RT_DEV float quad_child_key(float nx, float ny, float nz, float fx, float fy, float fz, const Ray& r, V inv, float tmin,
+                            float tmax_entry, float pb, float dmi) {
+    const float tnx = (nx - r.o.x) * inv.x, tfx = (fx - r.o.x) * inv.x;
+    const float tny = (ny - r.o.y) * inv.y, tfy = (fy - r.o.y) * inv.y;
+    const float tnz = (nz - r.o.z) * inv.z, tfz = (fz - r.o.z) * inv.z;
+    const float lo = __builtin_fmaxf(__builtin_fmaxf(tnx, tny), __builtin_fmaxf(tnz, tmin));
+    const float hi = __builtin_fminf(__builtin_fminf(tfx, tfy), __builtin_fminf(tfz, tmax_entry));
+    const float te = lo - dmi;
+    const bool go = lo <= hi && te <= pb;
+    return go ? __builtin_fminf(te, 3.4028235e38f) : kInf;
+}
+RT_DEV bool quad_sort_push(float key, uint32_t child, uint32_t k, uint32_t* qs, uint32_t& sp, uint32_t& cur) {
+    const float k1 = quad_perm<kQuadRot1>(key), k2 = quad_perm<kQuadRot2>(key), k3 = quad_perm<kQuadRot3>(key);
+    const uint32_t rank = ((k1 < key || (k1 == key && k >= 3u)) ? 1u : 0u) + ((k2 < key || (k2 == key && k >= 2u)) ? 1u : 0u) +
+                          ((k3 < key || (k3 == key && k >= 1u)) ? 1u : 0u);
+    const uint32_t others = (k1 != kInf ? 1u : 0u) + (k2 != kInf ? 1u : 0u) + (k3 != kInf ? 1u : 0u);
+    const bool vis = key != kInf;
+    if (vis && rank != 0u) {
+        const uint32_t at = (sp + others - rank) * 128u;
+        qs[at] = child;
+        qs[at + 64u] = __float_as_uint(key);
+    }
+    uint32_t nearest = vis && rank == 0u ? child : 0u;
+    nearest |= quad_perm<kQuadXor1>(nearest);
+    nearest |= quad_perm<kQuadRot2>(nearest);
+    const uint32_t n = others + (vis ? 1u : 0u);
+    if (n == 0u) return false;
+    cur = nearest;
+    sp += n - 1u;
+    return true;
+}
+[[maybe_unused]] __shared__ uint32_t quad_map[32];
+#ifdef RT_LEAF_AUDIT
+__device__ unsigned long long g_quad_iters;
+#endif
+template <uint32_t kF>
+RT_DEV void bvh_quad_tail(const DevScene& S, float delta, const f4* wrapper, const Ray& r, V inv, float tmin,
+                          float& closest, uint32_t& hit_code, uint32_t* stk, uint32_t mode, Trav& tv, bool live) {
+    PROF_T0(prep);
+    const uint32_t lane = __lane_id(), k = lane & 3u;
+    const uint64_t m = __ballot(1), L = __ballot(live);
+    const uint64_t H = m & (m >> 1) & (m >> 2) & (m >> 3) & 0x1111111111111111ull;
+    const uint32_t nlive = (uint32_t)__popcll(L);
+    const auto below = [](uint64_t x) {
+        return __builtin_amdgcn_mbcnt_hi((uint32_t)(x >> 32), __builtin_amdgcn_mbcnt_lo((uint32_t)x, 0u));
+    };
+    const auto pull = [](uint32_t from, uint32_t v) {
+        return (uint32_t)__builtin_amdgcn_ds_bpermute((int)(from << 2), (int)v);
+    };
+    const auto pullf = [&](uint32_t from, float v) { return __uint_as_float(pull(from, __float_as_uint(v))); };
+    const uint32_t live_rank = below(L), h0_rank = below(H);
+    const bool h0 = ((uint32_t)(H >> lane) & 1u) != 0u;
+    if (live && live_rank < 16u) quad_map[live_rank] = lane;
+    if (h0 && h0_rank < 16u) quad_map[16u + h0_rank] = lane;
+    __builtin_amdgcn_wave_barrier();
+    const bool host_quad = ((uint32_t)(H >> (lane & 60u)) & 1u) != 0u;
+    const uint32_t hq = below(H << 3);
+    const bool hosting = host_quad && hq < nlive && hq < 16u;
+    const uint32_t owner = hosting ? (quad_map[hq & 15u] & 63u) : lane;
+    const uint32_t my_host = live ? (quad_map[16u + (live_rank & 15u)] & 63u) : kNoNode;
+    __builtin_amdgcn_wave_barrier();
+    Ray q;
+    q.o = mk(pullf(owner, r.o.x), pullf(owner, r.o.y), pullf(owner, r.o.z));
+    q.d = mk(pullf(owner, r.d.x), pullf(owner, r.d.y), pullf(owner, r.d.z));
+    q.time = (kF & kFLeafRM) != 0u ? pullf(owner, r.time) : 0.0f;
+    const V qi = mk(pullf(owner, inv.x), pullf(owner, inv.y), pullf(owner, inv.z));
+    float qc = pullf(owner, closest);
+    const float qtmax = pullf(owner, tv.tmax_entry);
+    uint32_t cur = pull(owner, tv.cur), sp = pull(owner, tv.sp), brank = pull(owner, tv.best_rank);
+    uint32_t hcode = pull(owner, hit_code);
+    uint32_t any_u = pull(owner, tv.any ? 1u : 0u);
+    if (!hosting) cur = kNoNode;
+    uint32_t* qs = stk + owner - lane;
+    const bool prune = (__float_as_uint(ld4c(wrapper + 7).w) & rtdev::kBvhPrunable) != 0u ||
+                       (kPruneAllExpBuild && (mode & kModePruneAllExp));
+    const float dmi = delta * fmaxf(fmaxf(__builtin_fabsf(qi.x), __builtin_fabsf(qi.y)), __builtin_fabsf(qi.z));
+    PROF_ADD(kPrQuadRepack, prep);
+    [[maybe_unused]] uint32_t iters = 0u;
+    for (;;) {
+        const bool alive = cur != kNoNode;
+        const uint64_t am = __ballot(alive);
+        if (am == 0ull) break;
+        PROF_LIVE_ITER(2u, (uint32_t)__popcll(am) / 4u);
+        PROF_T0(pq);
+#ifdef RT_LEAF_AUDIT
+        if (alive && k == 0u) iters += 1u;
+        if (alive && ((cur & ~rtdev::kLeafNodeFlag) >= S.num_nodes || sp > S.stack_depth + S.spill_depth)) {
+            atomicAdd(&g_bounds_audit_count, 1u);
+            cur = kNoNode;
+            continue;
+        }
+#endif
+        uint32_t msx, msy, msz;
+        asm volatile("v_ashrrev_i32 %0, 31, %1" : "=v"(msx) : "v"(qi.x));
+        asm volatile("v_ashrrev_i32 %0, 31, %1" : "=v"(msy) : "v"(qi.y));
+        asm volatile("v_ashrrev_i32 %0, 31, %1" : "=v"(msz) : "v"(qi.z));
+        const uint32_t onx = msx & 48u, ony = (msy & 48u) + 16u, onz = (msz & 48u) + 32u;
+        const bool leaf = alive && (cur & rtdev::kLeafNodeFlag) != 0u;
+        if (__ballot(leaf) != 0ull) {
+            if (leaf && k == 0u) {
+                bool qany = any_u != 0u;
+                leaf_node_visit<kF>(S, delta, cur, onx, ony, onz, prune && !(mode & kModeNoLeafBoxes), qtmax, q, qi, tmin,
+                                    qc, brank, hcode, qany, mode);
+                any_u = qany ? 1u : 0u;
+            }
+            qc = quad_perm<kQuadLane0>(qc);
+            brank = quad_perm<kQuadLane0>(brank);
+            hcode = quad_perm<kQuadLane0>(hcode);
+            any_u = quad_perm<kQuadLane0>(any_u);
+        }
+        float key = kInf;
+        uint32_t child = rtdev::kChildEmpty;
+        if (alive && !leaf) {
+            const uint32_t nbo = cur * (rtdev::kBvhNodeF4 * 16u) + 4u * k;
+            const f4* nd = S.nodes;
+            const float nx = ld1_at(nd, nbo + onx), ny = ld1_at(nd, nbo + ony), nz = ld1_at(nd, nbo + onz),
+                        fx = ld1_at(nd, nbo + (onx ^ 48u)), fy = ld1_at(nd, nbo + (ony ^ 80u)),
+                        fz = ld1_at(nd, nbo + (onz ^ 112u));
+            child = __float_as_uint(ld1_at(nd, nbo + 96u));
+            key = quad_child_key(nx, ny, nz, fx, fy, fz, q, qi, tmin, qtmax, prune ? prune_bound(qc) : kInf,
+                                 prune ? dmi : 0.0f);
+        }
+        uint32_t next = kNoNode;
+        const bool went = quad_sort_push(key, child, k, qs, sp, next);
+        if (alive) {
+            if (!went) {
+                while (sp > 0u) {
+                    sp -= 1u;
+                    const uint32_t cand = qs[sp * 128u];
+                    const float tenter = __uint_as_float(qs[sp * 128u + 64u]);
+                    if (!prune || !(tenter > prune_bound(qc))) {
+                        next = cand;
+                        break;
+                    }
+                }
+            }
+            cur = next;
+        }
+        PROF_ADD(kPrQuadIter, pq);
+    }
+    PROF_LIVE_ITER(2u, 0u);
+    PROF_T0(pun);
+#ifdef RT_LEAF_AUDIT
+    if (iters) atomicAdd(&g_quad_iters, (unsigned long long)iters);
+#endif
+    const float rc = pullf(my_host, qc);
+    const uint32_t rh = pull(my_host, hcode), rb = pull(my_host, brank), ra = pull(my_host, any_u);
+    if (my_host != kNoNode) {
+        closest = rc;
+        hit_code = rh;
+        tv.best_rank = rb;
+        tv.any = ra != 0u;
+        tv.sp = 0u;
+    }
+    PROF_ADD(kPrQuadRepack, pun);
 }
 
 RT_DEV Ray apply_op(f4 op, Ray r) {
@@ -1450,7 +1601,7 @@
     return r;
 }
 constexpr uint32_t kRunPretestMin = 8u;
-template <int kKind, uint32_t kF>
+template <int kKind, uint32_t kF, bool kTopWalk = false>
 RT_DEV bool entry_geom_hit(const DevScene& S, float delta, const DevEntry* E, Ray r, float tmin, float& closest,
                            uint32_t& hit_code, uint32_t* stk, uint32_t mode, bool& replay) {
     uint32_t ntf = uni<kF>(cst(E)->ntf);
@@ -1526,8 +1677,8 @@
             ABLATE(kAbBvh2, float c2 = closest; uint32_t h2 = 0u; bool rp = false;
                    if (bvh_hit<kKind, kF>(S, delta, cst(E)->payload, r, tmin, c2, h2, stk, mode, rp) && h2 == 0x7fffffffu)
                        closest = -1.0f;);
-            return bvh_hit<kKind, kF>(S, delta, uni<kF>(cst(E)->payload), r, tmin, closest, hit_code, stk, mode,
-                                            replay);
+            return bvh_hit<kKind, kF, kTopWalk>(S, delta, uni<kF>(cst(E)->payload), r, tmin, closest, hit_code, stk, mode,
+                                                replay);
         }
     }
     if constexpr (kUniformEntries<kF>) {
@@ -2070,6 +2221,7 @@
     for (uint32_t e = 0; e < S.num_top; ++e) {
         const DevEntry* E = S.entries + e;
         PROF_T0(pe);
+        PROF_ENTRY(e);
         if (uni<kF>(cst(E)->kind) == rtdev::kEntMedium) {
             float t, vb = kInf;
             if constexpr (kKind == 0 && kMediumFirst<kF>) {
@@ -2089,7 +2241,7 @@
             }
         } else {
             uint32_t code;
-            if (entry_geom_hit<kKind, kF>(S, delta, E, r, 0.001f, closest, code, stk, mode, replay)) {
+            if (entry_geom_hit<kKind, kF, true>(S, delta, E, r, 0.001f, closest, code, stk, mode, replay)) {
                 hit_entry = e;
                 hit_code = code;
                 any = true;
@@ -2115,6 +2267,7 @@
     for (uint32_t e = 0; e < S.num_top; ++e) {
         if (!(active && w.pos == e)) continue;
         PROF_T0(pe);
+        PROF_ENTRY(e);
         const DevEntry* E = S.entries + e;
         const uint32_t kind = uni<kF>(cst(E)->kind);
         if (kind == rtdev::kEntMedium) {
@@ -2512,7 +2665,8 @@
 #ifdef RT_CAMMEM
     const DevCamera& Cs = *reinterpret_cast<const DevCamera*>(reinterpret_cast<const char*>(ctr) + kCamOffset);
 #else
-    const DevCamera& Cs = C;
+    const DevCamera& Cs =
+        kQuadTail<kKind, kF> ? *reinterpret_cast<const DevCamera*>(reinterpret_cast<const char*>(ctr) + kCamOffset) : C;
 #endif
     unsigned* counter = &ctr->batch;
     const ReplayItem* list = nullptr;
@@ -2766,6 +2920,80 @@
     }
     out[2u * i] = r0;
     out[2u * i + 1u] = r1;
+}
+
+__global__ __launch_bounds__(64) void kat_quad(const float* __restrict__ in, float* __restrict__ out, uint32_t n) {
+    __shared__ uint32_t ks[2u * 4u * 128u];
+    const uint32_t lane = threadIdx.x, k = lane & 3u, cs = blockIdx.x * 16u + lane / 4u;
+    if (cs >= n) return;
+    const float* a = in + 40u * cs;
+    uint32_t* o = reinterpret_cast<uint32_t*>(out) + 24u * cs;
+    Ray r;
+    r.o = mk(a[28], a[29], a[30]);
+    r.d = mk(a[31], a[32], a[33]);
+    r.time = 0.0f;
+    const V inv = mk(1.0f / r.d.x, 1.0f / r.d.y, 1.0f / r.d.z);
+    const float tmin = a[34], tmax_entry = a[35], closest = a[36], delta = a[38];
+    const bool prune = a[37] != 0.0f;
+    const float dmi = delta * fmaxf(fmaxf(__builtin_fabsf(inv.x), __builtin_fabsf(inv.y)), __builtin_fabsf(inv.z));
+    const float pb = prune ? prune_bound(closest) : kInf, dm = prune ? dmi : 0.0f;
+    const uint32_t sx = inv.x < 0.0f ? 12u : 0u, sy = inv.y < 0.0f ? 12u : 0u, sz = inv.z < 0.0f ? 12u : 0u;
+    for (uint32_t i = 0; i < 8u; ++i) {
+        ks[i * 128u + lane] = 0xdeadbeefu;
+        ks[i * 128u + 64u + lane] = 0xdeadbeefu;
+    }
+    __builtin_amdgcn_wave_barrier();
+    {
+        const float key = quad_child_key(a[sx + k], a[4u + sy + k], a[8u + sz + k], a[12u - sx + k], a[16u - sy + k],
+                                         a[20u - sz + k], r, inv, tmin, tmax_entry, pb, dm);
+        uint32_t sp = 1u, cur = 0xffffffffu;
+        uint32_t* qs = ks + (lane & 60u);
+        const bool went = quad_sort_push(key, __float_as_uint(a[24u + k]), k, qs, sp, cur);
+        __builtin_amdgcn_wave_barrier();
+        o[k] = __float_as_uint(key);
+        if (k == 0u) {
+            o[8] = sp;
+            o[9] = went ? cur : 0xffffffffu;
+            for (uint32_t i = 0; i < 3u; ++i) {
+                o[10u + i] = qs[(1u + i) * 128u];
+                o[13u + i] = qs[(1u + i) * 128u + 64u];
+            }
+        }
+    }
+    if (k == 0u) {
+        const auto row = [&](uint32_t b) { return f4{a[b], a[b + 1u], a[b + 2u], a[b + 3u]}; };
+        float key[4];
+        child_keys4_nf(row(sx), row(4u + sy), row(8u + sz), row(12u - sx), row(16u - sy), row(20u - sz), r, inv, tmin,
+                       tmax_entry, pb, dm, key);
+        float t0 = key[0], t1 = key[1], t2 = key[2], t3 = key[3];
+        uint32_t c0 = __float_as_uint(a[24]), c1 = __float_as_uint(a[25]), c2 = __float_as_uint(a[26]),
+                 c3 = __float_as_uint(a[27]);
+        for (uint32_t i = 0; i < 4u; ++i) o[4u + i] = __float_as_uint(key[i]);
+        uint32_t sp = 1u, cur = 0xffffffffu;
+        uint32_t* stk = ks + 512u + lane;
+        auto push = [&](uint32_t node, float t) {
+            stk[sp * 128u] = node;
+            stk[sp * 128u + 64u] = __float_as_uint(t);
+            sp += 1u;
+        };
+        sort2(t0, c0, t1, c1);
+        sort2(t2, c2, t3, c3);
+        sort2(t0, c0, t2, c2);
+        sort2(t1, c1, t3, c3);
+        sort2(t1, c1, t2, c2);
+        if (t0 != kInf) {
+            if (t3 != kInf) push(c3, t3);
+            if (t2 != kInf) push(c2, t2);
+            if (t1 != kInf) push(c1, t1);
+            cur = c0;
+        }
+        o[16] = sp;
+        o[17] = cur;
+        for (uint32_t i = 0; i < 3u; ++i) {
+            o[18u + i] = stk[(1u + i) * 128u];
+            o[21u + i] = stk[(1u + i) * 128u + 64u];
+        }
+    }
 }
 
 }
@@ -3108,6 +3336,16 @@
             fprintf(stderr, "]}\n");
         }
         {
+            fprintf(stderr, "{\"live_hist\": {\"bins\": %u, \"rows\": %u, \"classes\": [", kLiveBins, kLiveRows);
+            for (uint32_t c = 0; c < kLiveClasses; ++c) {
+                fprintf(stderr, "%s[", c ? "," : "");
+                for (uint32_t i = 0; i < kLiveRows * kLiveBins; ++i)
+                    fprintf(stderr, "%s%llu", i ? "," : "", h[kProfLive0 + c * kLiveRows * kLiveBins + i]);
+                fprintf(stderr, "]");
+            }
+            fprintf(stderr, "]}}\n");
+        }
+        {
             const unsigned long long* th = h + 3u * kPrCount;
             fprintf(stderr, "{\"trips_hist\": [%llu,%llu,%llu,%llu,%llu,%llu,%llu,%llu], \"wave_max_hist\": "
                             "[%llu,%llu,%llu,%llu,%llu,%llu,%llu,%llu]}\n",
@@ -3199,6 +3437,9 @@
         }
         if (hipMemcpyFromSymbol(&na, HIP_SYMBOL(g_bounds_audit_count), sizeof na) == hipSuccess)
             fprintf(stderr, "{\"bounds_audit_count\": %u}\n", na);
+        unsigned long long nq = 0;
+        if (hipMemcpyFromSymbol(&nq, HIP_SYMBOL(g_quad_iters), sizeof nq) == hipSuccess)
+            fprintf(stderr, "{\"quad_iters\": %llu}\n", nq);
 #endif
         if (s->done) (void)hipEventSynchronize(s->done);
         if (s->pool) (void)hipFree(s->pool);
@@ -3794,20 +4035,23 @@
 int rt_device_kat(int op, const float* in, float* out, uint32_t n) {
     rthost::clear_error();
     if (!in || !out) return rthost::set_error(RT_ERR_INVALID, "NULL argument");
-    if (op < 0 || op > 4) return rthost::set_error(RT_ERR_INVALID, "unknown KAT op");
+    if (op < 0 || op > 5) return rthost::set_error(RT_ERR_INVALID, "unknown KAT op");
     int rc = check_device(0);
     if (rc) return rc;
     if (n == 0) return RT_OK;
     DeviceGuard g(0);
-    const size_t in_floats = (size_t)n * (op <= 1 ? 14u : (op == 2 || op == 4 ? 3u : 12u)),
-                 out_floats = (size_t)n * 2u;
+    const size_t in_floats = (size_t)n * (op == 5 ? 40u : op <= 1 ? 14u : (op == 2 || op == 4 ? 3u : 12u)),
+                 out_floats = (size_t)n * (op == 5 ? 24u : 2u);
     float *din = nullptr, *dout = nullptr;
     hipError_t e = hipMalloc(&din, in_floats * sizeof(float));
     if (e == hipSuccess) e = hipMalloc(&dout, out_floats * sizeof(float));
     if (e == hipSuccess) e = hipMemcpy(din, in, in_floats * sizeof(float), hipMemcpyHostToDevice);
     if (e == hipSuccess) {
         (void)hipGetLastError();
-        hipLaunchKernelGGL(kat_eval, dim3((n + 63u) / 64u), dim3(64), 0, nullptr, op, din, dout, n);
+        if (op == 5)
+            hipLaunchKernelGGL(kat_quad, dim3((n + 15u) / 16u), dim3(64), 0, nullptr, din, dout, n);
+        else
+            hipLaunchKernelGGL(kat_eval, dim3((n + 63u) / 64u), dim3(64), 0, nullptr, op, din, dout, n);
         e = hipGetLastError();
     }
     if (e == hipSuccess) e = hipMemcpy(out, dout, out_floats * sizeof(float), hipMemcpyDeviceToHost);
diff --git a/raytracinginoneweekendinrust_amd/csrc/leaf_node_body.inc b/raytracinginoneweekendinrust_amd/csrc/leaf_node_body.inc
--- /dev/null
+++ b/raytracinginoneweekendinrust_amd/csrc/leaf_node_body.inc
@@ -0,0 +1,74 @@
+            const uint32_t nbo = (lnode & ~rtdev::kLeafNodeFlag) * (rtdev::kBvhNodeF4 * 16u);
+            const f4* nd = S.nodes;
+            const float2 nx2 = ld2_at(nd, nbo + onx), ny2 = ld2_at(nd, nbo + ony), nz2 = ld2_at(nd, nbo + onz),
+                         fx2 = ld2_at(nd, nbo + (onx ^ 48u)), fy2 = ld2_at(nd, nbo + (ony ^ 80u)),
+                         fz2 = ld2_at(nd, nbo + (onz ^ 112u)), chs = ld2_at(nd, nbo + 96u), rks = ld2_at(nd, nbo + 112u);
+            float tmr = tmax_entry, nt = 0.0f;
+            bool nh = false;
+            uint32_t ncode = 0u, nrank = 0u;
+            const uint32_t nleaf = __float_as_uint(chs.y) == rtdev::kChildEmpty ? 1u : 2u;
+            float llo[2] = {-kInf, -kInf}, lhi[2] = {kInf, kInf};
+            if (leaf_boxes) leaf_intervals2_nf(nx2, ny2, nz2, fx2, fy2, fz2, r, inv, delta, llo, lhi);
+            for (uint32_t k = 0; k < nleaf; ++k) {
+                const uint32_t lcode = __float_as_uint(k ? chs.y : chs.x), rank = __float_as_uint(k ? rks.y : rks.x);
+#ifdef RT_LEAF_AUDIT
+                const float2 bx0 = ld2(S.nodes + nbo / 16u, 0), by0 = ld2(S.nodes + nbo / 16u, 1),
+                             bz0 = ld2(S.nodes + nbo / 16u, 2), bx1 = ld2(S.nodes + nbo / 16u, 3),
+                             by1 = ld2(S.nodes + nbo / 16u, 4), bz1 = ld2(S.nodes + nbo / 16u, 5);
+                const float x0 = k ? bx0.y : bx0.x, y0 = k ? by0.y : by0.x, z0 = k ? bz0.y : bz0.x;
+                const float x1 = k ? bx1.y : bx1.x, y1 = k ? by1.y : by1.x, z1 = k ? bz1.y : bz1.x;
+#endif
+                const float bound = tmr < closest ? tmr : closest;
+                if (!leaf_boxes || leaf_interval_may_hit(k ? llo[1] : llo[0], k ? lhi[1] : lhi[0], tmin, bound)) {
+                    PROF_T0(pl);
+                    const float cap = closest < kInf ? __uint_as_float(__float_as_uint(closest) + 1u) : kInf;
+                    float c = tmr < cap ? tmr : cap;
+                    uint32_t code = 0u;
+                    const RayD q = to_d(r);
+                    ABLATE(kAbLeaf2, float c2 = c; uint32_t h2 = 0u;
+                           if (leaf_hit<kF>(S, lcode, r, q, tmin, c2, h2) && h2 == 0x7fffffffu) c = -1.0f;);
+                    bool hit;
+                    if constexpr (kLeafEmbed<kF>) {
+                        const uint32_t ltype = rtdev::leaf_type(lcode);
+                        const uint32_t lo = nbo + 4u * k;
+                        if (ltype == rtdev::kLeafSphere) {
+                            const f4 sp{ld1_at(nd, lo + 8u), ld1_at(nd, lo + 24u), ld1_at(nd, lo + 40u), ld1_at(nd, lo + 104u)};
+                            float ts;
+                            hit = sphere_t(sp, q, tmin, c, ts);
+                            if (hit) {
+                                c = ts;
+                                code = lcode;
+                            }
+                        } else if (ltype == rtdev::kLeafCube) {
+                            hit = cube_hit<(kF & kFTri) == 0u>(S, rtdev::leaf_index(lcode), ld1_at(nd, lo), ld1_at(nd, lo + 16u),
+                                                               ld1_at(nd, lo + 32u), ld1_at(nd, lo + 48u), ld1_at(nd, lo + 64u),
+                                                               ld1_at(nd, lo + 80u), r, inv, tmin, c, code);
+                        } else {
+                            hit = leaf_hit<kF, (kF & kFTri) == 0u, false, true>(S, lcode, r, q, tmin, c, code, inv);
+                        }
+                    } else {
+                        hit = leaf_hit<kF, (kF & kFTri) == 0u>(S, lcode, r, q, tmin, c, code, inv);
+                    }
+                    if (hit) {
+                        const uint32_t rk = rank + (rtdev::leaf_type(lcode) == rtdev::kLeafCube
+                                                        ? rtdev::leaf_index(code) - rtdev::leaf_index(lcode)
+                                                        : 0u);
+                        if (!nh || !(nt < c)) {
+                            nh = true;
+                            nt = c;
+                            ncode = code;
+                            nrank = rk;
+                        }
+                        tmr = c;
+                    }
+                    PROF_ADD(kPrLeafTest, pl);
+                } else {
+                    LEAF_AUDIT(lcode, rank, x0, y0, z0, x1, y1, z1);
+                }
+            }
+            if (nh && (nt < closest || (nt == closest && nrank > best_rank))) {
+                closest = nt;
+                best_rank = nrank;
+                hit_code = ncode;
+                any = true;
+            }
```

New measurement: 1321 Msamples/s (median of 6 runs). 3.1% higher.
